# nmonette/TO-UED

Measured on NVIDIA B200. Metric: gridworld agent env-steps/sec incl. LPG update, higher is better.
Workload: dtype f16/bf16 operands, f32 accumulate (GRU); f32 elsewhere

## Files before the change

__graft_entry__.py:

```python
import os
import sys

ROOT = os.path.dirname(os.path.abspath(__file__))
if ROOT not in sys.path:
    sys.path.insert(0, ROOT)


def build() -> None:
    from to_ued_b200.csrc.build import build as _build
    path = _build(verbose=False)
    _build(verbose=False, variant="fuzz")
    import to_ued_b200
    from to_ued_b200 import _lib
    assert os.path.exists(path) and _lib.lib().toued_version() >= 1


def smoke() -> None:
    import numpy as np
    import torch
    sys.path.insert(0, os.path.join(ROOT, "tests"))
    from helpers import Case, to_oracle_traj, rel_err
    from oracle import prng
    from oracle.agents import AgentTables
    from oracle.meta import lpg_meta_grad_train_step as o_step
    from to_ued_b200.meta.train import lpg_meta_grad_train_step, LPGTrainState, _WS_CACHE
    from to_ued_b200.models.lpg import LPG
    from to_ued_b200.models.optim import Adam
    from to_ued_b200.util.data import LpgHyperparams, TrainState

    assert torch.cuda.is_available(), "smoke() needs cuda:0"
    torch.cuda.set_device(0)
    K, n = 2, 2
    c = Case("all_shortlife", n=n, seed=1, table_scale=0.3)
    ag, ro = c.agent_state()
    ts = LPGTrainState(LPG(), torch.from_numpy(c.lpg).cuda(), Adam(1e-4))
    vc = TrainState(Case.pad8(c.value), torch.zeros(n, dtype=torch.int32, device="cuda"), 1, 4e0, 0.5)
    hy = LpgHyperparams(K, 0.5, 5e-2, 1e-3, 5e-3, 1e-3)
    new_ts, ag2, vc2, met = lpg_meta_grad_train_step(prng.PRNGKey(3), ts, ag, vc, ro, 1, 0.99, 0.95, hy, return_grad=True)
    torch.cuda.synchronize()
    tape = list(_WS_CACHE.values())[0].tape
    trajs = [to_oracle_traj(tape.transition(k)) for k in range(K)]
    ev = to_oracle_traj(tape.transition(K))
    s0 = c.oro.batch_reset(None, c.p, c.w)
    rngs = prng.split(prng.PRNGKey(3), n)
    r_train = prng.split(rngs, 2)[:, 1, :]
    r0 = prng.split(r_train, 2)[:, 1, :]
    otraj, _, _ = c.oro.batch_rollout(r0, c.actor, c.p, s0)
    assert (otraj.action == trajs[0].action).all() and (otraj.obs_idx == trajs[0].obs_idx).all(), "rollout parity"
    dt = torch.float64
    oag = AgentTables(torch.tensor(c.actor).to(dt), torch.tensor(c.critic).to(dt), torch.zeros(n, dtype=torch.long))
    o = o_step(prng.PRNGKey(3), c.layout, torch.tensor(c.lpg).to(dt), oag, torch.tensor(c.value).to(dt), c.oro, c.p,
               s0, c.life, num_agent_updates=K, trajectories=trajs, eval_trajectory=ev, do_eval=False)
    err = rel_err(met["_grad"].cpu().numpy(), o["grad"].numpy())
    import to_ued_b200
    tol = 2e-2 if to_ued_b200.GRU_PRECISION == "tc" else 2e-4
    assert err < tol, f"meta-gradient mismatch vs oracle: {err}"
    print(f"smoke ok: rollout bit-exact, meta-gradient rel err {err:.2e}, lpg_loss {float(met['lpg_loss']):.5f}")


if __name__ == "__main__":
    build()
    if "--smoke" in sys.argv:
        smoke()
```

include/toued.h:

```cpp
#ifndef TOUED_H
#define TOUED_H
#include <stdint.h>
#ifdef __cplusplus
extern "C" {
#endif

#define TOUED_LEVEL_BYTES 192

const char* toued_last_error(void);
int toued_version(void);

int toued_rollout(const void* levels, const uint32_t* keys, const float* actor,
                  const uint8_t* forced_actions, int32_t* state, int32_t* obs, uint8_t* action,
                  float* reward, uint8_t* done, float* ep_return, int n_agents, int n_workers,
                  int rollout_len, int obs_dim, int max_grid_size, int max_n_objs, int reset_first,
                  void* stream);

int toued_env_step(const void* levels, const uint32_t* keys, const int32_t* actions, int32_t* state,
                   int32_t* obs, float* reward, uint8_t* done, int n_agents, int n_workers,
                   int max_grid_size, int max_n_objs, void* stream);
int toued_env_reset(const void* levels, int32_t* state, int32_t* obs, int n_agents, int n_workers,
                    int max_grid_size, void* stream);


int toued_sort_tokens(const int32_t* obs, uint16_t* sorted_tok, int n_agents, int n_workers,
                      int rollout_len, void* stream);

int toued_lpg_prepare(const int32_t* obs, const uint8_t* action, const float* reward,
                      const uint8_t* done, const float* actor, const float* critic,
                      const float* lpg_params, const int32_t* step, const void* levels, float* x,
                      void* ximg, int n_agents, int n_workers, int rollout_len, int obs_dim,
                      int lifetime_conditioning, int lpg_stride, void* stream);

int toued_gru_forward(const float* x, const uint8_t* done, const float* lpg_params, float* h_out,
                      float* gates, float* pi_hat, float* y_hat, int n_agents, int n_workers,
                      int rollout_len, int lifetime_conditioning, int lpg_stride, void* stream);

int toued_agent_scratch_floats(int n_agents, int n_workers, int rollout_len, int obs_dim);
int toued_agent_update(const int32_t* obs, const uint8_t* action, const uint16_t* sorted_tok,
                       const float* pi_hat, const float* y_hat, const float* actor_in,
                       const float* critic_in, float* actor_out, float* critic_out,
                       const void* levels, int32_t* step, float* scalars, int n_agents,
                       int n_workers, int rollout_len, int obs_dim, float lr_actor, float lr_critic,
                       float max_grad_norm, float agent_target_coeff, int tables_precopied, float* run_scratch,
                       void* stream);


int toued_meta_loss(const int32_t* obs, const uint8_t* action, const float* reward,
                    const uint8_t* done, const uint16_t* sorted_tok, const float* value_table,
                    const float* actor, float* lam, float* mu, float* scalars, int n_agents,
                    int n_workers, int rollout_len, int obs_dim, int value_stride, float gamma,
                    float gae_lambda, float grad_scale, int outer_product_quirk, void* stream);

int toued_agent_backward(const int32_t* obs, const uint8_t* action, const uint16_t* sorted_tok,
                         const float* pi_hat, const float* y_hat, const float* actor_k,
                         const float* critic_k, const float* actor_k1, const float* critic_k1,
                         const float* update_scalars, float* lam, float* mu, float* d_pi_hat,
                         float* d_y_hat, int n_agents, int n_workers, int rollout_len, int obs_dim,
                         float lr_actor, float lr_critic, float max_grad_norm,
                         float agent_target_coeff, float policy_entropy_coeff,
                         float target_entropy_coeff, float policy_l2_coeff, float target_l2_coeff,
                         float grad_scale, float* run_scratch, void* stream);

int toued_transpose_wh(const float* lpg_params, float* whT, void* stream);

int toued_gru_backward(const uint8_t* done, const float* lpg_params, const float* whT,
                       const float* h, float* gates, const float* y_hat, const float* d_pi_hat,
                       const float* d_y_hat, float* dl, float* dx, int n_agents, int n_workers,
                       int rollout_len, int lifetime_conditioning, void* stream);

int toued_lpg_wgrad_workspace_floats(void);
int toued_lpg_wgrad(const int32_t* obs, const uint8_t* done, const float* critic,
                    const float* lpg_params, const float* x, const float* h, const float* dgates,
                    const float* d_pi_hat, const float* dl, const float* dx, float* workspace,
                    int n_agents, int n_workers, int rollout_len, int obs_dim,
                    int lifetime_conditioning, int accumulate, void* stream);
int toued_lpg_wgrad_workspace_offset(int which);
int toued_lpg_wgrad_embed(const int32_t* obs, const uint8_t* done, const float* critic, const float* lpg_params,
                          const float* dx, float* workspace, const uint32_t* cotangent_max, int n_agents, int n_workers,
                          int rollout_len, int obs_dim, int lifetime_conditioning, int accumulate, void* stream);
int toued_lpg_wgrad_splits(int which);
int toued_reduce_partials(const float* workspace, float* grad, int lifetime_conditioning, int wh_splits,
                          int sm_splits, void* stream);

int toued_adam(float* params, const float* grad, float* mu, float* nu, int n, int count, float lr,
               float b1, float b2, float eps, void* stream);
int toued_adam_dev(float* params, const float* grad, float* mu, float* nu, int* count_dev, int n, float lr,
                   float b1, float b2, float eps, void* stream);
int toued_sgd_clip(float* params, const float* grad, float* sqnorm_scratch, int n, float lr, float max_norm,
                   void* stream);

int toued_a2c_update(const int32_t* obs, const uint8_t* action, const float* reward, const uint8_t* done,
                     const uint16_t* sorted_tok, const float* actor_in, const float* critic_in,
                     float* actor_out, float* critic_out, const void* levels, int32_t* step,
                     float* scalars, int n_agents, int n_workers, int rollout_len, int obs_dim,
                     float lr_actor, float lr_critic, float max_grad_norm, float gamma, float gae_lambda,
                     float entropy_coeff, int outer_product_quirk, void* stream);

int toued_a2c_train(const void* levels, const uint32_t* keys, float* actor0, float* actor1, float* critic0,
                    float* critic1, int32_t* state, int32_t* obs, uint8_t* action, float* reward, uint8_t* done,
                    uint16_t* sorted_tok, int32_t* step, float* scalars, float* loss_sums, int num_updates,
                    int n_agents, int n_workers, int rollout_len, int obs_dim, int max_grid_size, int max_n_objs,
                    float lr_actor, float lr_critic, float max_grad_norm, float gamma, float gae_lambda,
                    float entropy_coeff, int outer_product_quirk, void* stream);

int toued_es_ask(const uint32_t* key, const float* mean, float sigma, float* candidates, int popsize,
                 int n_params, int cand_stride, void* stream);
int toued_es_tell(const float* candidates, const float* fitness, float* mean, float* m, float* v,
                  int popsize, int n_params, int cand_stride, float sigma, float lrate, float beta1,
                  float beta2, float eps, int gen_counter, float mean_decay, void* stream);

int toued_es_ask_shard(const uint32_t* key, const float* mean, float sigma, float* candidates, int popsize_global,
                       int n_params, int cand_stride, int pair_offset, int n_pairs, void* stream);
int toued_es_grad_partial(const float* candidates, const float* fitness, const float* mean, float* grad_sum,
                          int n_members, int n_params, int cand_stride, float sigma, void* stream);
int toued_es_adam(const float* grad_sum, float* mean, float* m, float* v, int popsize_global, int n_params,
                  float sigma, float lrate, float beta1, float beta2, float eps, int gen_counter, float mean_decay,
                  void* stream);

int toued_plr_reset_lowest(float* score, uint8_t* active, uint8_t* is_new, int buffer_size, int minimum_new,
                           int* reset_ids, void* stream);
int toued_plr_select(uint32_t key0, uint32_t key1, float* score, uint8_t* active, uint8_t* is_new, int buffer_size,
                     const int* old_ids, const uint8_t* terminated, const float* new_scores, int n_agents,
                     float p_replay, float temperature, int shuffle_rounds, int* new_ids, void* stream);

int toued_generate_levels_desc_bytes(void);
int toued_generate_levels(const void* gen_desc, const uint32_t* keys, const int32_t* buffer_ids, void* levels_out,
                          int32_t* lifetimes_out, int n_levels, void* stream);

int toued_get_nash(const float* game, const float* x0, const float* y0, float* x_out, float* y_out,
                   int n, int x_nz, int y_nz, int num_iters, float lr, void* stream);
int toued_projection_simplex(float* v, int n, int max_nz, void* stream);


int toued_init_tables(const uint32_t* keys, const uint8_t* mask, float* tables, int n_agents,
                      int obs_dim, int n_out, void* stream);
int toued_masked_reset(const void* levels, const uint8_t* mask, int32_t* state, int32_t* obs,
                       int32_t* step, int n_agents, int n_workers, int max_grid_size, void* stream);

int toued_host_iota_bits(const uint32_t* keys, int n_keys, int n, uint32_t* out);


int toued_key_split(const uint32_t* keys_in, int n_keys, int num, int offset, int count, uint32_t* out,
                    void* stream);
int toued_key_chain(const uint32_t* keys_in, int n_keys, int chain_len, uint32_t* keys_out,
                    uint32_t* carry_out, void* stream);


int toued_tc_gemm_test(const float* A, const float* B, void* scratch_img, float* D, void* stream);
int toued_tc_gemm_mixed_test(const float* A, const float* B, void* scratch_img, float* D, void* stream);
int toued_tc_gemm_mn_test(const float* A, const float* B, void* scratch_img, float* D, int lbo, int sbo,
                          int kadv, void* stream);
int toued_tc_gemm_mn2_test(const float* A, const float* B, void* scratch_img, float* D, void* stream);

int toued_pack_wh_forward(const float* lpg_params, void* wh_img, int lifetime_conditioning, void* stream);
int toued_gru_forward_tc(const float* x, const uint8_t* done, const float* lpg_params, const void* wh_img,
                         void* h16, void* fac, void* hpimg, float* pi_hat, float* y_hat, int n_agents,
                         int n_workers, int rollout_len, int lifetime_conditioning, void* stream);
int toued_pack_wh_forward_multi(const float* lpg_params, void* wh_img, int lifetime_conditioning, int n_sets,
                                int lpg_stride, void* stream);
int toued_gru_forward_tc_multi(const float* x, const uint8_t* done, const float* lpg_params, const void* wh_img,
                               float* pi_hat, float* y_hat, int n_agents, int n_workers, int rollout_len,
                               int lifetime_conditioning, int lpg_stride, void* stream);

int toued_pack_wh_backward(const float* lpg_params, void* whb_img, void* stream);
#define TOUED_STATUS_NONFINITE_COT 1u
#define TOUED_STATUS_FP16_RANGE 2u
int toued_cotangent_max(const float* d_pi_hat, const float* d_y_hat, int n_agents, int n_workers, int rollout_len,
                        uint32_t* cotangent_max, void* stream);
int toued_gru_backward_tc(const uint8_t* done, const float* lpg_params, const void* whb_img,
                          const void* h16, const void* fac, const float* y_hat, const float* d_pi_hat,
                          const float* d_y_hat, void* dgimg, float* dl, float* dx, uint32_t* cotangent_max,
                          int n_agents, int n_workers, int rollout_len, int lifetime_conditioning, void* stream);
int toued_wgrad_tc_splits(void);
int toued_wgrad_tc_small_splits(void);
int toued_lpg_wgrad_tc(const void* hpimg, const void* dgimg, const void* ximg, const void* h16,
                       const float* d_pi_hat, const float* dl, float* wh_partials, float* small_partials,
                       uint32_t* cotangent_max, int n_agents, int n_workers, int rollout_len, int accumulate,
                       void* stream);

#ifdef __cplusplus
}
#endif
#endif
```

to_ued_b200/_lib.py:

```python
from __future__ import annotations

import ctypes as C
import os

_HERE = os.path.dirname(os.path.abspath(__file__))
_VARIANT = os.environ.get("TOUED_LIB_VARIANT", "")
LIB_PATH = os.path.join(_HERE, f"libtoued_{_VARIANT}.so" if _VARIANT else "libtoued.so")

_lib = None


class TouedError(RuntimeError):
    pass


def lib() -> C.CDLL:
    global _lib
    if _lib is None:
        if not os.path.exists(LIB_PATH):
            raise TouedError(
                f"{LIB_PATH} is missing: the CUDA extension is not built. "
                "Run `python -m to_ued_b200.csrc.build` (there is no CPU fallback).")
        _lib = C.CDLL(LIB_PATH)
        _declare(_lib)
    return _lib


_P, _I, _F = C.c_void_p, C.c_int, C.c_float

SIGNATURES = {
    "toued_rollout": [_P] * 10 + [_I] * 7 + [_P],
    "toued_env_step": [_P] * 7 + [_I] * 4 + [_P],
    "toued_env_reset": [_P] * 3 + [_I] * 3 + [_P],
    "toued_sort_tokens": [_P] * 2 + [_I] * 3 + [_P],
    "toued_lpg_prepare": [_P] * 11 + [_I] * 6 + [_P],
    "toued_gru_forward": [_P] * 7 + [_I] * 5 + [_P],
    "toued_agent_update": [_P] * 12 + [_I] * 4 + [_F] * 4 + [_I, _P, _P],
    "toued_agent_scratch_floats": [_I] * 4,
    "toued_meta_loss": [_P] * 10 + [_I] * 5 + [_F] * 3 + [_I, _P],
    "toued_agent_backward": [_P] * 14 + [_I] * 4 + [_F] * 9 + [_P, _P],
    "toued_transpose_wh": [_P] * 3,
    "toued_gru_backward": [_P] * 10 + [_I] * 4 + [_P],
    "toued_lpg_wgrad_workspace_floats": [],
    "toued_lpg_wgrad": [_P] * 11 + [_I] * 6 + [_P],
    "toued_reduce_partials": [_P, _P, _I, _I, _I, _P],
    "toued_lpg_wgrad_splits": [_I],
    "toued_lpg_wgrad_workspace_offset": [_I],
    "toued_lpg_wgrad_embed": [_P] * 7 + [_I] * 6 + [_P],
    "toued_cotangent_max": [_P, _P, _I, _I, _I, _P, _P],
    "toued_pack_wh_backward": [_P] * 3,
    "toued_gru_backward_tc": [_P] * 12 + [_I] * 4 + [_P],
    "toued_wgrad_tc_splits": [],
    "toued_wgrad_tc_small_splits": [],
    "toued_lpg_wgrad_tc": [_P] * 9 + [_I] * 4 + [_P],
    "toued_adam": [_P] * 4 + [_I, _I] + [_F] * 4 + [_P],
    "toued_adam_dev": [_P] * 5 + [_I] + [_F] * 4 + [_P],
    "toued_sgd_clip": [_P] * 3 + [_I, _F, _F, _P],
    "toued_get_nash": [_P] * 5 + [_I] * 4 + [_F, _P],
    "toued_projection_simplex": [_P, _I, _I, _P],
    "toued_es_ask": [_P, _P, _F, _P, _I, _I, _I, _P],
    "toued_es_tell": [_P] * 5 + [_I, _I, _I] + [_F] * 5 + [_I, _F, _P],
    "toued_es_ask_shard": [_P, _P, _F, _P, _I, _I, _I, _I, _I, _P],
    "toued_es_grad_partial": [_P] * 4 + [_I, _I, _I, _F, _P],
    "toued_es_adam": [_P] * 4 + [_I, _I] + [_F] * 5 + [_I, _F, _P],
    "toued_a2c_update": [_P] * 12 + [_I] * 4 + [_F] * 6 + [_I, _P],
    "toued_a2c_train": [_P] * 15 + [_I] * 7 + [_F] * 6 + [_I, _P],
    "toued_init_tables": [_P] * 3 + [_I] * 3 + [_P],
    "toued_masked_reset": [_P] * 5 + [_I] * 3 + [_P],
    "toued_generate_levels_desc_bytes": [],
    "toued_generate_levels": [_P] * 5 + [_I, _P],
    "toued_plr_reset_lowest": [_P] * 3 + [_I, _I, _P, _P],
    "toued_plr_select": [C.c_uint32, C.c_uint32] + [_P] * 3 + [_I] + [_P] * 3 + [_I, _F, _F, _I, _P, _P],
    "toued_tc_gemm_test": [_P] * 5,
    "toued_tc_gemm_mixed_test": [_P] * 5,
    "toued_tc_gemm_mn_test": [_P] * 4 + [_I] * 3 + [_P],
    "toued_tc_gemm_mn2_test": [_P] * 5,
    "toued_pack_wh_forward": [_P, _P, _I, _P],
    "toued_pack_wh_forward_multi": [_P, _P, _I, _I, _I, _P],
    "toued_gru_forward_tc_multi": [_P] * 6 + [_I] * 5 + [_P],
    "toued_host_iota_bits": [_P, _I, _I, _P],
    "toued_key_split": [_P, _I, _I, _I, _I, _P, _P],
    "toued_key_chain": [_P, _I, _I, _P, _P, _P],
    "toued_gru_forward_tc": [_P] * 9 + [_I] * 4 + [_P],
}


def _declare(l):
    l.toued_last_error.restype = C.c_char_p
    l.toued_last_error.argtypes = []
    l.toued_version.restype = _I
    l.toued_version.argtypes = []
    for name, args in SIGNATURES.items():
        fn = getattr(l, name)
        fn.restype = _I
        fn.argtypes = args


def ptr(t):
    if t is None:
        return None
    if not t.is_cuda:
        raise TouedError("to_ued_b200 ops need CUDA tensors (there is no CPU fallback)")
    if not t.is_contiguous():
        raise TouedError("to_ued_b200 ops need contiguous tensors")
    return t.data_ptr()


def stream_ptr():
    import torch
    return torch.cuda.current_stream().cuda_stream


KERNELS_PER_CALL = {"toued_adam_dev": 2, "toued_sgd_clip": 2, "toued_lpg_wgrad": 3, "toued_init_tables": 2, "toued_lpg_wgrad_tc": 2, "toued_pack_wh_forward": 2, "toued_pack_wh_forward_multi": 2}
LAUNCHES = {}
GRAPH_KERNELS = [0]
ENV_STEPS = [0]
PROFILE = None


H2D_BYTES = [0]


def h2d(t):
    H2D_BYTES[0] += int(t.numel() * t.element_size()) if hasattr(t, "element_size") else int(t.nbytes)
    return t


def reset_counters(profile=False):
    global PROFILE
    H2D_BYTES[0] = 0
    GRAPH_KERNELS[0] = 0
    ENV_STEPS[0] = 0
    LAUNCHES.clear()
    PROFILE = {} if profile else None


def kernel_launches():
    return sum(n * KERNELS_PER_CALL.get(k, 1) for k, n in LAUNCHES.items()) + GRAPH_KERNELS[0]


def profile_ms():
    return {k: (len(v), sum(a.elapsed_time(b) for a, b in v)) for k, v in (PROFILE or {}).items()}


def call(name, *args):
    LAUNCHES[name] = LAUNCHES.get(name, 0) + 1
    if name == "toued_rollout":
        ENV_STEPS[0] += args[10] * args[11] * args[12]
    elif name == "toued_a2c_train":
        ENV_STEPS[0] += args[15] * args[16] * args[17] * args[18]
    if PROFILE is not None:
        import torch
        a, b = torch.cuda.Event(enable_timing=True), torch.cuda.Event(enable_timing=True)
        a.record()
        rc = getattr(lib(), name)(*args)
        b.record()
        PROFILE.setdefault(name, []).append((a, b))
    else:
        rc = getattr(lib(), name)(*args)
    if rc != 0:
        raise TouedError(f"{name} failed ({rc}): {lib().toued_last_error().decode()}")
```

to_ued_b200/agents/lpg_agent.py:

```python
from __future__ import annotations

from dataclasses import dataclass, field
from typing import Any, List, Optional

import numpy as np
import torch

from .. import _lib
from ..util import prng
from ..util.data import AgentState, Transition


@dataclass
class LPGAgentMetrics:
    policy_l2: Any
    policy_entropy: Any
    critic_loss: Any
    critic_l2: Any
    critic_entropy: Any

    def as_dict(self):
        return {"policy_l2": self.policy_l2, "policy_entropy": self.policy_entropy,
                "critic_loss": self.critic_loss, "critic_l2": self.critic_l2,
                "critic_entropy": self.critic_entropy}


class Tape:

    def __init__(self, n_agents, n_workers, rollout_len, obs_dim, num_updates, device, keep_gates=True,
                 precision=None, per_agent_params=False):
        import to_ued_b200
        N, W, L, D, K = n_agents, n_workers, rollout_len, obs_dim, num_updates
        R, dev = N * W, device
        f32, u8, i32 = torch.float32, torch.uint8, torch.int32
        self.N, self.W, self.L, self.D, self.K, self.R = N, W, L, D, K, R
        self.record = bool(keep_gates)
        kt = K + 1 if self.record else 2
        kr = K + 1 if self.record else 1
        ka = K if self.record else 1
        self.kt, self.kr, self.ka = kt, kr, ka
        self.actor = torch.empty((kt, N, D, 8), dtype=f32, device=dev)
        self.critic = torch.empty((kt, N, D, 8), dtype=f32, device=dev)
        self.obs = torch.empty((kr, N, L + 1, W), dtype=i32, device=dev)
        self.action = torch.empty((kr, N, L, W), dtype=u8, device=dev)
        self.reward = torch.empty((kr, N, L, W), dtype=f32, device=dev)
        self.done = torch.empty((kr, N, L, W), dtype=u8, device=dev)
        self.sorted_tok = torch.empty((kr, N, L * W), dtype=torch.int16, device=dev)
        self.precision = precision or to_ued_b200.GRU_PRECISION
        self.x = torch.empty((ka, L, R, 8), dtype=f32, device=dev)
        self.ximg = None
        if self.precision == "tc":
            f16 = torch.float16
            Rp = (R + 63) // 64 * 64
            R32 = (R + 31) // 32 * 32
            self.h16 = None if per_agent_params else torch.empty((ka, L, R32, 256), dtype=f16, device=dev)
            self.fac = torch.empty((ka, 4, L, R32, 256), dtype=f16, device=dev) if self.record else None
            self.hpimg = torch.zeros((ka, L * Rp * 256 * 2), dtype=torch.uint8, device=dev) if self.record else None
            self.ximg = torch.zeros((ka, L * Rp * 128), dtype=torch.uint8, device=dev) if self.record else None
            self.wh_img = torch.zeros((N if per_agent_params else 1) * 16 * 26624 // 2, dtype=f16, device=dev)
            self.h = self.gates = None
        else:
            self.h = torch.empty((ka, L, R, 256), dtype=f32, device=dev)
            self.gates = torch.empty((ka, 4, L, R, 256), dtype=f32, device=dev) if self.record else None
        self.pi_hat = torch.empty((ka, L, R), dtype=f32, device=dev)
        self.y_hat = torch.empty((ka, L, R, 8), dtype=f32, device=dev)
        self.scalars = torch.empty((ka, N, 8), dtype=f32, device=dev)
        self.scal_sum = torch.zeros((N, 8), dtype=f32, device=dev)
        self.step_in = torch.empty((ka, N), dtype=i32, device=dev)
        self.ep_return = torch.empty((N, W), dtype=f32, device=dev)
        self.agent_scratch = torch.empty(_lib.lib().toued_agent_scratch_floats(N, W, L, D), dtype=f32, device=dev)

    def ti(self, k):
        return k if self.record else (k & 1)

    def ri(self, k):
        return k if self.record else 0

    def ai(self, k):
        return k if self.record else 0

    def transition(self, k) -> Transition:
        r = self.ri(k)
        return Transition(self.obs[r], self.action[r], self.reward[r], self.done[r])


_SORT_STREAMS = {}


def _sort_stream(cur):
    key = (cur.device.index, cur.cuda_stream)
    st = _SORT_STREAMS.get(key)
    if st is None:
        st = _SORT_STREAMS[key] = torch.cuda.Stream(device=cur.device)
    return st


def _mark(label):
    import to_ued_b200
    if to_ued_b200.PHASE_EVENTS is not None and getattr(to_ued_b200, "PHASE_FINE", False):
        e = torch.cuda.Event(enable_timing=True)
        e.record(torch.cuda.current_stream())
        to_ued_b200.PHASE_EVENTS.append((label, -2, e))


def lpg_agent_train_step(k, tape: Tape, levels, step, lpg_params, lifetime_conditioning, agent_target_coeff,
                         lr_actor, lr_critic, max_grad_norm, lpg_stride=0):
    N, W, L, D = tape.N, tape.W, tape.L, tape.D
    s = _lib.stream_ptr()
    p = _lib.ptr
    r, a, t0, t1 = tape.ri(k), tape.ai(k), tape.ti(k), tape.ti(k + 1)
    import to_ued_b200
    cur = torch.cuda.current_stream()
    side = _sort_stream(cur) if to_ued_b200.SIDE_STREAMS else cur
    ev_roll, ev_sort = torch.cuda.Event(), torch.cuda.Event()
    ev_roll.record(cur)
    with torch.cuda.stream(side):
        side.wait_event(ev_roll)
        _lib.call("toued_sort_tokens", p(tape.obs[r]), p(tape.sorted_tok[r]), N, W, L, _lib.stream_ptr())
        precopied = bool(to_ued_b200.SIDE_STREAMS)
        if precopied:
            tape.actor[t1].copy_(tape.actor[t0])
            tape.critic[t1].copy_(tape.critic[t0])
        ev_sort.record(side)
    _mark("rollout")
    tape.step_in[a].copy_(step)
    _lib.call("toued_lpg_prepare", p(tape.obs[r]), p(tape.action[r]), p(tape.reward[r]), p(tape.done[r]),
              p(tape.actor[t0]), p(tape.critic[t0]), p(lpg_params), p(step), p(levels), p(tape.x[a]),
              p(tape.ximg[a]) if tape.ximg is not None else None,
              N, W, L, D, int(lifetime_conditioning), int(lpg_stride), s)
    if lpg_stride and tape.precision == "tc":
        _lib.call("toued_gru_forward_tc_multi", p(tape.x[a]), p(tape.done[r]), p(lpg_params), p(tape.wh_img),
                  p(tape.pi_hat[a]), p(tape.y_hat[a]), N, W, L, int(lifetime_conditioning), int(lpg_stride), s)
    elif lpg_stride or tape.precision != "tc":
        _lib.call("toued_gru_forward", p(tape.x[a]), p(tape.done[r]), p(lpg_params), p(tape.h[a]),
                  p(tape.gates[a]) if tape.gates is not None else None, p(tape.pi_hat[a]), p(tape.y_hat[a]),
                  N, W, L, int(lifetime_conditioning), int(lpg_stride), s)
    else:
        _lib.call("toued_gru_forward_tc", p(tape.x[a]), p(tape.done[r]), p(lpg_params), p(tape.wh_img),
                  p(tape.h16[a]), p(tape.fac[a]) if tape.fac is not None else None,
                  p(tape.hpimg[a]) if tape.hpimg is not None else None, p(tape.pi_hat[a]), p(tape.y_hat[a]),
                  N, W, L, int(lifetime_conditioning), s)
    _mark("gru_fwd")
    cur.wait_event(ev_sort)
    _mark("sort_wait")
    _lib.call("toued_agent_update", p(tape.obs[r]), p(tape.action[r]), p(tape.sorted_tok[r]), p(tape.pi_hat[a]),
              p(tape.y_hat[a]), p(tape.actor[t0]), p(tape.critic[t0]), p(tape.actor[t1]), p(tape.critic[t1]),
              p(levels), p(step), p(tape.scalars[a]), N, W, L, D, float(lr_actor), float(lr_critic),
              float(max_grad_norm), float(agent_target_coeff), int(precopied), p(tape.agent_scratch), s)
    tape.scal_sum += tape.scalars[a]
    _mark("update")


def train_lpg_agent_steps(rng, lpg_train_state, agent_state: AgentState, rollout_manager, num_train_steps: int,
                          agent_target_coeff: float, tape: Optional[Tape] = None, lpg_stride: int = 0):
    env = rollout_manager.env
    actor, critic = agent_state.actor_state, agent_state.critic_state
    N, W = agent_state.env_state.packed.shape
    L, K = rollout_manager.train_rollout_len, num_train_steps
    dev = actor.params.device
    if tape is None:
        import to_ued_b200
        tape = Tape(N, W, L, env.obs_dim, K, dev, keep_gates=False,
                    precision=to_ued_b200.ES_PRECISION if lpg_stride else None, per_agent_params=bool(lpg_stride))
    levels = agent_state.level.packed
    step = actor.step.clone()
    state = agent_state.env_state.packed.clone()
    tape.actor[0].copy_(actor.params)
    tape.critic[0].copy_(critic.params)
    tape.scal_sum.zero_()
    keys_d = prng.chain_device(prng.to_device(rng, dev), K)
    p = _lib.ptr
    lpg = lpg_train_state.params if hasattr(lpg_train_state, "params") else lpg_train_state
    cond = lpg_train_state.model.lifetime_conditioning if hasattr(lpg_train_state, "model") else False
    if tape.precision == "tc" and not lpg_stride:
        _lib.call("toued_pack_wh_forward", p(lpg), p(tape.wh_img), int(cond), _lib.stream_ptr())
    elif tape.precision == "tc":
        _lib.call("toued_pack_wh_forward_multi", p(lpg), p(tape.wh_img), int(cond), N, int(lpg_stride), _lib.stream_ptr())
    yield
    for k in range(K):
        r = tape.ri(k)
        _lib.call("toued_rollout", p(levels), p(keys_d[k]), p(tape.actor[tape.ti(k)]), None, p(state), p(tape.obs[r]),
                  p(tape.action[r]), p(tape.reward[r]), p(tape.done[r]), None, N, W, L, env.obs_dim,
                  env.max_grid_size, env.max_n_objs, 0, _lib.stream_ptr())
        lpg_agent_train_step(k, tape, levels, step, lpg, cond, agent_target_coeff, actor.learning_rate,
                             critic.learning_rate, actor.max_grad_norm, lpg_stride=lpg_stride)
        yield
    sc = tape.scal_sum / K
    metrics = LPGAgentMetrics(policy_l2=sc[:, 4], policy_entropy=sc[:, 6], critic_loss=sc[:, 3],
                              critic_l2=sc[:, 5], critic_entropy=sc[:, 7])
    from ..environments.gridworld.gridworld import EnvState
    new_agent = agent_state.replace(
        actor_state=actor.replace(params=tape.actor[tape.ti(K)].clone(), step=step),
        critic_state=critic.replace(params=tape.critic[tape.ti(K)].clone(), step=step.clone()),
        env_obs=tape.obs[tape.ri(K - 1)][:, -1].clone(), env_state=EnvState(state, env.max_n_objs))
    rollouts = [tape.transition(k) for k in range(K)] if tape.record else [tape.transition(K - 1)]
    return new_agent, rollouts, metrics


def train_lpg_agent(rng, lpg_train_state, agent_state: AgentState, rollout_manager, num_train_steps: int,
                    agent_target_coeff: float, tape: Optional[Tape] = None, lpg_stride: int = 0):
    gen = train_lpg_agent_steps(rng, lpg_train_state, agent_state, rollout_manager, num_train_steps,
                                agent_target_coeff, tape=tape, lpg_stride=lpg_stride)
    while True:
        try:
            next(gen)
        except StopIteration as done:
            return done.value
```

to_ued_b200/csrc/agent_backward.cu:

```cuda
#include "lpg_common.cuh"
#include "segreduce.cuh"
#include "../../include/toued.h"

__global__ void __launch_bounds__(256)
meta_loss_kernel(const int32_t* __restrict__ obs, const uint8_t* __restrict__ action,
                 const float* __restrict__ reward, const uint8_t* __restrict__ done,
                 const uint16_t* __restrict__ sorted_tok, const float* __restrict__ value,
                 const float* __restrict__ actor, float* __restrict__ lam, float* __restrict__ mu,
                 float* __restrict__ scal, int W, int L, int D, int vstride, float gamma, float lmbda,
                 float gscale, int quirk) {
    extern __shared__ __align__(16) float sm[];
    float* adv = sm;
    float* rec = adv + L * W;
    float* abar = rec + L * W * 6;
    float* lbar = abar + W;
    float* runv = lbar + W;
    float* scan = runv + L * W * 5;
    void* idxmem = scan + 2 * 256 * 5;
    __shared__ float red[32];
    __shared__ int iscan[512];
    __shared__ unsigned char sflags[512];
    const int n = blockIdx.x, tid = threadIdx.x, T = W * L;
    const int32_t* ob = obs + (size_t)n * (L + 1) * W;
    const uint8_t* act = action + (size_t)n * T;
    const float* rw = reward + (size_t)n * T;
    const uint8_t* dn = done + (size_t)n * T;
    const uint16_t* st = sorted_tok + (size_t)n * T;
    const float* vt = value + (size_t)n * D * vstride;
    const float* at = actor + (size_t)n * D * 8;
    float* lm = lam + (size_t)n * D * 8;
    float* mm = mu + (size_t)n * D * 8;
    const float invT = 1.0f / (float)T;
    const SegIndex si = seg_index_build(idxmem, iscan, st, ob, T);

    for (int i = tid; i < D * 2; i += 256) {
        reinterpret_cast<float4*>(lm)[i] = make_float4(0.f, 0.f, 0.f, 0.f);
        reinterpret_cast<float4*>(mm)[i] = make_float4(0.f, 0.f, 0.f, 0.f);
    }
    float s1 = 0.f, s2 = 0.f;
    const float vlast = vt[(size_t)(D - 1) * vstride];
    for (int w = tid; w < W; w += 256) {
        float g = 0.f;
        int32_t o1 = ob[L * W + w];
        float v1 = vt[(size_t)ob_idx(o1) * vstride] + 0.001f * (float)ob_time(o1) * vlast;
        for (int t = L - 1; t >= 0; --t) {
            const int32_t o0 = ob[t * W + w];
            const float v0 = vt[(size_t)ob_idx(o0) * vstride] + 0.001f * (float)ob_time(o0) * vlast;
            const float nd = dn[t * W + w] ? 0.0f : 1.0f;
            const float delta = rw[t * W + w] + gamma * v1 * nd - v0;
            g = delta + gamma * lmbda * nd * g;
            adv[t * W + w] = g;
            s1 += g; s2 = fmaf(g, g, s2);
            v1 = v0;
        }
    }
    s1 = block_sum(s1, red); s2 = block_sum(s2, red);
    const float mean = s1 * invT;
    float var = 0.f;
    for (int i = tid; i < T; i += 256) { const float d = adv[i] - mean; var = fmaf(d, d, var); }
    var = block_sum(var, red) * invT;
    const float inv_std = 1.0f / (sqrtf(var) + 1e-8f);
    __syncthreads();
    for (int i = tid; i < T; i += 256) adv[i] = (adv[i] - mean) * inv_std;
    __syncthreads();
    for (int tok = tid; tok < T; tok += 256) {
        const int32_t o = ob[tok];
        float z[5], p[5];
        tab_logits8<5>(at, D, o, z);
        softmax_c<5>(z, p);
        const int a = act[tok];
        float pa = p[0];
#pragma unroll
        for (int j = 1; j < 5; ++j) pa = (a == j) ? p[j] : pa;
        float* r = rec + tok * 6;
        r[5] = logf(pa + 1e-8f);
        const float q = pa / (pa + 1e-8f);
#pragma unroll
        for (int j = 0; j < 5; ++j) r[j] = q * ((a == j ? 1.0f : 0.0f) - p[j]);
    }
    __syncthreads();
    float loss = 0.f;
    for (int w = tid; w < W; w += 256) {
        float sa = 0.f, sl = 0.f, se = 0.f;
        for (int t = 0; t < L; ++t) { sa += adv[t * W + w]; sl += rec[(t * W + w) * 6 + 5]; se = fmaf(adv[t * W + w], rec[(t * W + w) * 6 + 5], se); }
        abar[w] = sa / (float)L; lbar[w] = sl / (float)L;
        loss -= quirk ? abar[w] * lbar[w] : se / (float)L;
    }
    loss = block_sum(loss, red) / (float)W;
    __syncthreads();
    float last[5] = {0.f, 0.f, 0.f, 0.f, 0.f};
    for (int tok = tid; tok < T; tok += 256) {
        const int w = tok % W;
        const float coef = -gscale * invT * (quirk ? abar[w] : adv[tok]);
        float* r = rec + tok * 6;
        const float tf = 0.001f * (float)ob_time(ob[tok]);
#pragma unroll
        for (int j = 0; j < 5; ++j) { r[j] *= coef; last[j] = fmaf(tf, r[j], last[j]); }
        r[5] = tf;
    }
#pragma unroll
    for (int j = 0; j < 5; ++j) last[j] = block_sum(last[j], red);
    __syncthreads();
    seg_reduce<5, 6>(rec, si, T, runv, scan, sflags);
    for (int r = tid; r < si.nruns; r += 256) {
        const int row = si.run_row[r];
#pragma unroll
        for (int j = 0; j < 5; ++j) lm[(size_t)row * 8 + j] = runv[r * 5 + j];
    }
    if (tid == 0) {
#pragma unroll
        for (int j = 0; j < 5; ++j) lm[(size_t)(D - 1) * 8 + j] = last[j];
        scal[n * 2 + 0] = loss;
        scal[n * 2 + 1] = s2 * invT;
    }
}

extern "C" int toued_meta_loss(const int32_t* obs, const uint8_t* action, const float* reward,
                               const uint8_t* done, const uint16_t* sorted_tok, const float* value_table,
                               const float* actor, float* lam, float* mu, float* scalars, int n_agents,
                               int n_workers, int rollout_len, int obs_dim, int value_stride, float gamma,
                               float gae_lambda, float grad_scale, int outer_product_quirk, void* stream) {
    const int T = n_workers * rollout_len;
    TOUED_CHECK(n_agents > 0 && T > 0, "toued_meta_loss: empty problem");
    const size_t smem = sizeof(float) * ((size_t)T * 7 + 2 * n_workers + (size_t)T * 5 + 2 * 256 * 5) + seg_index_bytes(T);
    TOUED_CHECK(smem <= 200 * 1024, "toued_meta_loss: W*L=%d too large for shared memory", T);
    TOUED_CUDA(cudaFuncSetAttribute(meta_loss_kernel, cudaFuncAttributeMaxDynamicSharedMemorySize, (int)smem));
    meta_loss_kernel<<<n_agents, 256, smem, (cudaStream_t)stream>>>(
        obs, action, reward, done, sorted_tok, value_table, actor, lam, mu, scalars, n_workers, rollout_len,
        obs_dim, value_stride, gamma, gae_lambda, grad_scale, outer_product_quirk);
    TOUED_LAUNCH_CHECK();
    return 0;
}

struct TokFwd { float p[5], y[8], pa, q, tf; int a; };

__device__ __forceinline__ TokFwd tok_forward(const float* at, const float* ct, int D, int32_t o, int a) {
    TokFwd f;
    float z[5], zy[8];
    tab_logits8<5>(at, D, o, z);
    softmax_c<5>(z, f.p);
    tab_logits8<8>(ct, D, o, zy);
    softmax_c<8>(zy, f.y);
    f.a = a;
    f.pa = f.p[0];
#pragma unroll
    for (int j = 1; j < 5; ++j) f.pa = (a == j) ? f.p[j] : f.pa;
    f.q = f.pa / (f.pa + 1e-8f);
    f.tf = 0.001f * (float)ob_time(o);
    return f;
}

__device__ __forceinline__ void tok_grad(const TokFwd& f, float ph, const float* yh, float invT, float alpha, float* c) {
    const float ca = invT * ph * f.q;
#pragma unroll
    for (int j = 0; j < 5; ++j) c[j] = ca * ((f.a == j ? 1.0f : 0.0f) - f.p[j]);
    float mm[8], b = 0.f;
#pragma unroll
    for (int i = 0; i < 8; ++i) {
        mm[i] = logf(f.y[i] + 1e-8f) - logf(yh[i] + 1e-8f) + f.y[i] / (f.y[i] + 1e-8f);
        b = fmaf(f.y[i], mm[i], b);
    }
    const float cc = alpha * invT;
#pragma unroll
    for (int i = 0; i < 8; ++i) c[5 + i] = cc * f.y[i] * (mm[i] - b);
}

__device__ __forceinline__ void load8(const float* p, float* v) {
    const float4 a = reinterpret_cast<const float4*>(p)[0], b = reinterpret_cast<const float4*>(p)[1];
    v[0] = a.x; v[1] = a.y; v[2] = a.z; v[3] = a.w; v[4] = b.x; v[5] = b.y; v[6] = b.z; v[7] = b.w;
}

__global__ void __launch_bounds__(256, 2)
agent_backward_kernel(const int32_t* __restrict__ obs, const uint8_t* __restrict__ action,
                      const uint16_t* __restrict__ sorted_tok, const float* __restrict__ pi_hat,
                      const float* __restrict__ y_hat, const float* __restrict__ actor_k,
                      const float* __restrict__ critic_k, const float* __restrict__ actor_k1,
                      const float* __restrict__ critic_k1, const float* __restrict__ upd_scal,
                      float* lam, float* mu, float* __restrict__ d_pi_hat, float* __restrict__ d_y_hat,
                      float* run_scratch, int n_agents, int W, int L, int D, float lr_a, float lr_c, float max_norm,
                      float alpha, float b_pent, float b_yent, float b_pl2, float b_yl2, float gscale) {
    extern __shared__ __align__(16) float rec[];
    __shared__ float red[32];
    __shared__ float s_wlast[13];
    __shared__ int iscan[512];
    __shared__ unsigned char sflags[512];
    const int n = blockIdx.x, tid = threadIdx.x, T = W * L, R = n_agents * W;
    const int32_t* ob = obs + (size_t)n * (L + 1) * W;
    const uint8_t* act = action + (size_t)n * T;
    const uint16_t* st = sorted_tok + (size_t)n * T;
    const float* a0 = actor_k + (size_t)n * D * 8;
    const float* c0 = critic_k + (size_t)n * D * 8;
    const float* a1 = actor_k1 + (size_t)n * D * 8;
    const float* c1 = critic_k1 + (size_t)n * D * 8;
    float* lm = lam + (size_t)n * D * 8;
    float* mm = mu + (size_t)n * D * 8;
    const float invT = 1.0f / (float)T;
    const float gna = upd_scal[n * 8 + 0], gnc = upd_scal[n * 8 + 1];
    const bool keep = upd_scal[n * 8 + 2] != 0.0f;
    float* runv = run_scratch + (size_t)n * min(T, D) * 13;
    float* scan = rec + (size_t)T * 13;
    const SegIndex si = seg_index_build(scan + 2 * 256 * 13, iscan, st, ob, T);

    float last[13];
#pragma unroll
    for (int j = 0; j < 13; ++j) last[j] = 0.f;
    for (int tok = tid; tok < T; tok += 256) {
        const TokFwd f = tok_forward(a1, c1, D, ob[tok], act[tok]);
        float* r = rec + tok * 13;
        {
            float dh[5], s = 0.f;
#pragma unroll
            for (int j = 0; j < 5; ++j) { dh[j] = -(logf(f.p[j] + 1e-8f) + 1.0f); s = fmaf(f.p[j], dh[j], s); }
            const float k = -b_pent * gscale * invT;
#pragma unroll
            for (int j = 0; j < 5; ++j) r[j] = k * f.p[j] * (dh[j] - s);
        }
        {
            float dh[8], s = 0.f;
#pragma unroll
            for (int j = 0; j < 8; ++j) { dh[j] = -(logf(f.y[j] + 1e-8f) + 1.0f); s = fmaf(f.y[j], dh[j], s); }
            const float k = -b_yent * gscale * invT;
#pragma unroll
            for (int j = 0; j < 8; ++j) r[5 + j] = k * f.y[j] * (dh[j] - s);
        }
#pragma unroll
        for (int j = 0; j < 13; ++j) last[j] = fmaf(f.tf, r[j], last[j]);
    }
#pragma unroll
    for (int j = 0; j < 13; ++j) last[j] = block_sum(last[j], red);
    __syncthreads();
    seg_reduce<13, 13>(rec, si, T, runv, scan, sflags);
    for (int r = tid; r < si.nruns; r += 256) {
        const int row = si.run_row[r];
        const float* g = runv + r * 13;
#pragma unroll
        for (int j = 0; j < 5; ++j) lm[(size_t)row * 8 + j] += g[j];
#pragma unroll
        for (int j = 0; j < 8; ++j) mm[(size_t)row * 8 + j] += g[5 + j];
    }
    if (tid == 0) {
#pragma unroll
        for (int j = 0; j < 5; ++j) lm[(size_t)(D - 1) * 8 + j] += last[j];
#pragma unroll
        for (int j = 0; j < 8; ++j) mm[(size_t)(D - 1) * 8 + j] += last[5 + j];
    }
    __syncthreads();

    const float dir_pi = gscale * b_pl2 * 2.0f * invT;
    const float dir_y = gscale * b_yl2 * 2.0f * invT;
    if (!keep) {
        for (int tok = tid; tok < T; tok += 256) {
            const int t = tok / W, w = tok - t * W;
            const size_t li = (size_t)t * R + (size_t)n * W + w;
            d_pi_hat[li] = dir_pi * pi_hat[li];
            float yh[8]; load8(y_hat + li * 8, yh);
            float4* o = reinterpret_cast<float4*>(d_y_hat + li * 8);
            o[0] = make_float4(dir_y * yh[0], dir_y * yh[1], dir_y * yh[2], dir_y * yh[3]);
            o[1] = make_float4(dir_y * yh[4], dir_y * yh[5], dir_y * yh[6], dir_y * yh[7]);
        }
        return;
    }

#pragma unroll
    for (int j = 0; j < 13; ++j) last[j] = 0.f;
    for (int tok = tid; tok < T; tok += 256) {
        const int t = tok / W, w = tok - t * W;
        const size_t li = (size_t)t * R + (size_t)n * W + w;
        const TokFwd f = tok_forward(a0, c0, D, ob[tok], act[tok]);
        float yh[8]; load8(y_hat + li * 8, yh);
        float* r = rec + tok * 13;
        tok_grad(f, pi_hat[li], yh, invT, alpha, r);
#pragma unroll
        for (int j = 0; j < 13; ++j) last[j] = fmaf(f.tf, r[j], last[j]);
    }
#pragma unroll
    for (int j = 0; j < 13; ++j) last[j] = block_sum(last[j], red);
    __syncthreads();
    seg_reduce<13, 13>(rec, si, T, runv, scan, sflags);
    float dot_a = 0.f, dot_c = 0.f;
    for (int r = tid; r < si.nruns; r += 256) {
        const int row = si.run_row[r];
        const float* g = runv + r * 13;
        float l8[8], m8[8];
        load8(lm + (size_t)row * 8, l8); load8(mm + (size_t)row * 8, m8);
#pragma unroll
        for (int j = 0; j < 5; ++j) dot_a = fmaf(g[j], l8[j], dot_a);
#pragma unroll
        for (int j = 0; j < 8; ++j) dot_c = fmaf(g[5 + j], m8[j], dot_c);
    }
    dot_a = block_sum(dot_a, red); dot_c = block_sum(dot_c, red);
    float ll[8], ml[8];
    load8(lm + (size_t)(D - 1) * 8, ll); load8(mm + (size_t)(D - 1) * 8, ml);
#pragma unroll
    for (int j = 0; j < 5; ++j) dot_a = fmaf(last[j], ll[j], dot_a);
#pragma unroll
    for (int j = 0; j < 8; ++j) dot_c = fmaf(last[5 + j], ml[j], dot_c);
    const bool clip_a = !(gna < max_norm), clip_c = !(gnc < max_norm);
    const float ka = -lr_a * (clip_a ? max_norm / gna : 1.0f), pa_ = clip_a ? dot_a / (gna * gna) : 0.0f;
    const float kc = -lr_c * (clip_c ? max_norm / gnc : 1.0f), pc_ = clip_c ? dot_c / (gnc * gnc) : 0.0f;
    if (tid == 0) {
#pragma unroll
        for (int j = 0; j < 5; ++j) s_wlast[j] = ka * (ll[j] - pa_ * last[j]);
#pragma unroll
        for (int j = 0; j < 8; ++j) s_wlast[5 + j] = kc * (ml[j] - pc_ * last[5 + j]);
    }
    __syncthreads();
    float wl[13];
#pragma unroll
    for (int j = 0; j < 13; ++j) wl[j] = s_wlast[j];

    for (int r = tid; r < si.nruns; r += 256) {
        const int row = si.run_row[r];
        float* g = runv + r * 13;
        float l8[8], m8[8];
        load8(lm + (size_t)row * 8, l8); load8(mm + (size_t)row * 8, m8);
#pragma unroll
        for (int j = 0; j < 5; ++j) g[j] = ka * (l8[j] - pa_ * g[j]);
#pragma unroll
        for (int j = 0; j < 8; ++j) g[5 + j] = kc * (m8[j] - pc_ * g[5 + j]);
    }
    __syncthreads();
    float hl[13];
#pragma unroll
    for (int j = 0; j < 13; ++j) hl[j] = 0.f;
    for (int pos = tid; pos < T; pos += 256) {
        const int tok = si.tok[pos];
        const int t = tok / W, w = tok - t * W;
        const size_t li = (size_t)t * R + (size_t)n * W + w;
        const TokFwd f = tok_forward(a0, c0, D, ob[tok], act[tok]);
        const float ph = pi_hat[li];
        float yh[8]; load8(y_hat + li * 8, yh);
        float* r = rec + tok * 13;
        const float* wr = runv + (size_t)si.run[pos] * 13;
        float v[13];
#pragma unroll
        for (int j = 0; j < 13; ++j) v[j] = fmaf(f.tf, wl[j], wr[j]);
        float va = v[0], pv = 0.f;
#pragma unroll
        for (int j = 1; j < 5; ++j) va = (f.a == j) ? v[j] : va;
#pragma unroll
        for (int j = 0; j < 5; ++j) pv = fmaf(f.p[j], v[j], pv);
        const float s = va - pv;
        d_pi_hat[li] = invT * f.q * s + dir_pi * ph;
        const float pe = f.pa + 1e-8f;
        const float c1_ = ph * invT * s * 1e-8f * f.pa / (pe * pe), c2_ = ph * invT * f.q;
        float h[13];
#pragma unroll
        for (int j = 0; j < 5; ++j)
            h[j] = c1_ * ((f.a == j ? 1.0f : 0.0f) - f.p[j]) - c2_ * f.p[j] * (v[j] - pv);
        float m[8], mp[8], av = 0.f, b = 0.f;
#pragma unroll
        for (int j = 0; j < 8; ++j) {
            const float ye = f.y[j] + 1e-8f;
            m[j] = logf(ye) - logf(yh[j] + 1e-8f) + f.y[j] / ye;
            mp[j] = (f.y[j] + 2e-8f) / (ye * ye);
            av = fmaf(v[5 + j], f.y[j], av);
            b = fmaf(f.y[j], m[j], b);
        }
        const float ca = alpha * invT;
        float dS[8], sy = 0.f, dyo[8];
#pragma unroll
        for (int j = 0; j < 8; ++j) {
            const float vc = v[5 + j];
            dyo[j] = ca * f.y[j] * (av - vc) / (yh[j] + 1e-8f) + dir_y * yh[j];
            dS[j] = vc * m[j] + vc * f.y[j] * mp[j] - vc * b - av * (m[j] + f.y[j] * mp[j]);
            sy = fmaf(f.y[j], dS[j], sy);
        }
#pragma unroll
        for (int j = 0; j < 8; ++j) h[5 + j] = ca * f.y[j] * (dS[j] - sy);
        float4* o = reinterpret_cast<float4*>(d_y_hat + li * 8);
        o[0] = make_float4(dyo[0], dyo[1], dyo[2], dyo[3]);
        o[1] = make_float4(dyo[4], dyo[5], dyo[6], dyo[7]);
#pragma unroll
        for (int j = 0; j < 13; ++j) { r[j] = h[j]; hl[j] = fmaf(f.tf, h[j], hl[j]); }
    }
#pragma unroll
    for (int j = 0; j < 13; ++j) hl[j] = block_sum(hl[j], red);
    __syncthreads();
    seg_reduce<13, 13>(rec, si, T, runv, scan, sflags);
    for (int r = tid; r < si.nruns; r += 256) {
        const int row = si.run_row[r];
        const float* g = runv + r * 13;
#pragma unroll
        for (int j = 0; j < 5; ++j) lm[(size_t)row * 8 + j] += g[j];
#pragma unroll
        for (int j = 0; j < 8; ++j) mm[(size_t)row * 8 + j] += g[5 + j];
    }
    if (tid == 0) {
#pragma unroll
        for (int j = 0; j < 5; ++j) lm[(size_t)(D - 1) * 8 + j] = ll[j] + hl[j];
#pragma unroll
        for (int j = 0; j < 8; ++j) mm[(size_t)(D - 1) * 8 + j] = ml[j] + hl[5 + j];
    }
}

extern "C" int toued_agent_backward(const int32_t* obs, const uint8_t* action, const uint16_t* sorted_tok,
                                    const float* pi_hat, const float* y_hat, const float* actor_k,
                                    const float* critic_k, const float* actor_k1, const float* critic_k1,
                                    const float* update_scalars, float* lam, float* mu, float* d_pi_hat,
                                    float* d_y_hat, int n_agents, int n_workers, int rollout_len, int obs_dim,
                                    float lr_actor, float lr_critic, float max_grad_norm,
                                    float agent_target_coeff, float policy_entropy_coeff,
                                    float target_entropy_coeff, float policy_l2_coeff, float target_l2_coeff,
                                    float grad_scale, float* run_scratch, void* stream) {
    const int T = n_workers * rollout_len;
    TOUED_CHECK(n_agents > 0 && T > 0, "toued_agent_backward: empty problem");
    TOUED_CHECK(run_scratch != nullptr, "toued_agent_backward: run_scratch (toued_agent_scratch_floats) is required");
    const size_t smem = sizeof(float) * ((size_t)T * 13 + 2 * 256 * 13) + seg_index_bytes(T);
    TOUED_CHECK(smem <= 200 * 1024, "toued_agent_backward: W*L=%d too large for shared memory", T);
    TOUED_CUDA(cudaFuncSetAttribute(agent_backward_kernel, cudaFuncAttributeMaxDynamicSharedMemorySize, (int)smem));
    TOUED_CUDA(cudaFuncSetAttribute(agent_backward_kernel, cudaFuncAttributePreferredSharedMemoryCarveout, 100));
    cudaStream_t st = (cudaStream_t)stream;
    agent_backward_kernel<<<n_agents, 256, smem, st>>>(
        obs, action, sorted_tok, pi_hat, y_hat, actor_k, critic_k, actor_k1, critic_k1, update_scalars, lam, mu,
        d_pi_hat, d_y_hat, run_scratch, n_agents, n_workers, rollout_len, obs_dim, lr_actor, lr_critic, max_grad_norm,
        agent_target_coeff, policy_entropy_coeff, target_entropy_coeff, policy_l2_coeff, target_l2_coeff, grad_scale);
    TOUED_LAUNCH_CHECK();
    return 0;
}
```

to_ued_b200/csrc/agent_update.cu:

```cuda
#include "lpg_common.cuh"
#include "segreduce.cuh"
#include "../../include/toued.h"

constexpr int AU_C = 13;

__global__ void __launch_bounds__(256, 2)
agent_update_kernel(const int32_t* __restrict__ obs, const uint8_t* __restrict__ action,
                    const uint16_t* __restrict__ sorted_tok, const float* __restrict__ pi_hat,
                    const float* __restrict__ y_hat, const float* __restrict__ actor_in,
                    const float* __restrict__ critic_in, float* actor_out, float* critic_out,
                    const LevelRec* __restrict__ levels, int32_t* __restrict__ step,
                    float* __restrict__ scal, float* run_scratch, int n_agents, int W, int L, int D,
                    float lr_a, float lr_c, float max_norm, float alpha, int tables_precopied) {
    extern __shared__ __align__(16) float smc[];
    __shared__ float red[32];
    __shared__ int iscan[512];
    __shared__ unsigned char sflags[512];
    const int n = blockIdx.x, tid = threadIdx.x, T = W * L, R = n_agents * W;
    float* runv = run_scratch + (size_t)n * min(T, D) * 13;
    float* scan = smc + (size_t)T * AU_C;
    void* idxmem = scan + 2 * 256 * 13;
    const int32_t* ob = obs + (size_t)n * (L + 1) * W;
    const uint8_t* act = action + (size_t)n * T;
    const float* a_in = actor_in + (size_t)n * D * 8;
    const float* c_in = critic_in + (size_t)n * D * 8;
    float* a_out = actor_out + (size_t)n * D * 8;
    float* c_out = critic_out + (size_t)n * D * 8;
    const float invT = 1.0f / (float)T;
    const SegIndex si = seg_index_build(idxmem, iscan, sorted_tok + (size_t)n * T, ob, T);

    if (!tables_precopied)
        for (int i = tid; i < D * 2; i += 256) {
            reinterpret_cast<float4*>(a_out)[i] = reinterpret_cast<const float4*>(a_in)[i];
            reinterpret_cast<float4*>(c_out)[i] = reinterpret_cast<const float4*>(c_in)[i];
        }

    float m_kl = 0.f, m_pi2 = 0.f, m_y2 = 0.f;
    float last[13];
#pragma unroll
    for (int j = 0; j < 13; ++j) last[j] = 0.f;
    for (int tok = tid; tok < T; tok += 256) {
        const int t = tok / W, w = tok - t * W;
        const size_t li = (size_t)t * R + (size_t)n * W + w;
        const int32_t o = ob[tok];
        float z[5], p[5], zy[8], y[8];
        tab_logits8<5>(a_in, D, o, z);
        softmax_c<5>(z, p);
        tab_logits8<8>(c_in, D, o, zy);
        softmax_c<8>(zy, y);
        const int a = act[tok];
        float pa = p[0];
#pragma unroll
        for (int j = 1; j < 5; ++j) pa = (a == j) ? p[j] : pa;
        const float ph = pi_hat[li];
        const float ca = invT * ph * (pa / (pa + 1e-8f));
        float* rec = smc + tok * AU_C;
#pragma unroll
        for (int j = 0; j < 5; ++j) rec[j] = ca * ((a == j ? 1.0f : 0.0f) - p[j]);
        float yh[8];
        { const float4* q = reinterpret_cast<const float4*>(y_hat + li * 8); const float4 q0 = q[0], q1 = q[1];
          yh[0] = q0.x; yh[1] = q0.y; yh[2] = q0.z; yh[3] = q0.w; yh[4] = q1.x; yh[5] = q1.y; yh[6] = q1.z; yh[7] = q1.w; }
        float mm[8], b = 0.f, kl = 0.f, y2 = 0.f;
#pragma unroll
        for (int i = 0; i < 8; ++i) {
            const float ly = logf(y[i] + 1e-8f), lh = logf(yh[i] + 1e-8f);
            mm[i] = ly - lh + y[i] / (y[i] + 1e-8f);
            b = fmaf(y[i], mm[i], b);
            kl = fmaf(y[i], ly - lh, kl);
            y2 = fmaf(yh[i], yh[i], y2);
        }
        const float cc = alpha * invT;
#pragma unroll
        for (int i = 0; i < 8; ++i) rec[5 + i] = cc * y[i] * (mm[i] - b);
        const float tf = 0.001f * (float)ob_time(o);
#pragma unroll
        for (int j = 0; j < 13; ++j) last[j] = fmaf(tf, rec[j], last[j]);
        m_kl += kl; m_pi2 = fmaf(ph, ph, m_pi2); m_y2 += y2;
    }
#pragma unroll
    for (int j = 0; j < 13; ++j) last[j] = block_sum(last[j], red);
    m_kl = block_sum(m_kl, red); m_pi2 = block_sum(m_pi2, red); m_y2 = block_sum(m_y2, red);
    __syncthreads();

    seg_reduce<13, AU_C>(smc, si, T, runv, scan, sflags);
    float na = 0.f, nc = 0.f;
    for (int r = tid; r < si.nruns; r += 256) {
        const float* g = runv + r * 13;
#pragma unroll
        for (int j = 0; j < 5; ++j) na = fmaf(g[j], g[j], na);
#pragma unroll
        for (int j = 5; j < 13; ++j) nc = fmaf(g[j], g[j], nc);
    }
    na = block_sum(na, red); nc = block_sum(nc, red);
#pragma unroll
    for (int j = 0; j < 5; ++j) na = fmaf(last[j], last[j], na);
#pragma unroll
    for (int j = 5; j < 13; ++j) nc = fmaf(last[j], last[j], nc);
    const float gna = sqrtf(na), gnc = sqrtf(nc);
    const float sa = gna < max_norm ? 1.0f : max_norm / gna;
    const float sc = gnc < max_norm ? 1.0f : max_norm / gnc;
    const int old_step = step[n];
    const bool keep = (old_step + 1) <= levels[n].lifetime;
    const float ua = keep ? lr_a * sa : 0.0f, uc = keep ? lr_c * sc : 0.0f;

    for (int r = tid; r < si.nruns; r += 256) {
        const int row = si.run_row[r];
        const float* g = runv + r * 13;
#pragma unroll
        for (int j = 0; j < 5; ++j) a_out[(size_t)row * 8 + j] = a_in[(size_t)row * 8 + j] - ua * g[j];
#pragma unroll
        for (int j = 0; j < 8; ++j) c_out[(size_t)row * 8 + j] = c_in[(size_t)row * 8 + j] - uc * g[5 + j];
    }
    if (tid == 0) {
#pragma unroll
        for (int j = 0; j < 5; ++j) a_out[(size_t)(D - 1) * 8 + j] = a_in[(size_t)(D - 1) * 8 + j] - ua * last[j];
#pragma unroll
        for (int j = 0; j < 8; ++j) c_out[(size_t)(D - 1) * 8 + j] = c_in[(size_t)(D - 1) * 8 + j] - uc * last[5 + j];
        step[n] = keep ? old_step + 1 : old_step;
    }
    __syncthreads();

    float ea = 0.f, ec = 0.f;
    for (int tok = tid; tok < T; tok += 256) {
        const int32_t o = ob[tok];
        float z[5], p[5], zy[8], y[8];
        tab_logits8<5>(a_out, D, o, z);
        softmax_c<5>(z, p);
        tab_logits8<8>(c_out, D, o, zy);
        softmax_c<8>(zy, y);
#pragma unroll
        for (int j = 0; j < 5; ++j) { const float q = p[j] + 1e-8f; ea -= q * logf(q); }
#pragma unroll
        for (int j = 0; j < 8; ++j) { const float q = y[j] + 1e-8f; ec -= q * logf(q); }
    }
    ea = block_sum(ea, red); ec = block_sum(ec, red);
    if (tid == 0) {
        float* s = scal + (size_t)n * 8;
        s[0] = gna; s[1] = gnc; s[2] = keep ? 1.0f : 0.0f;
        s[3] = m_kl * invT;
        s[4] = m_pi2 * invT;
        s[5] = m_y2 * invT;
        s[6] = ea * invT;
        s[7] = ec * invT;
    }
}

static size_t agent_smem_bytes(int T, int D) {
    return sizeof(float) * ((size_t)T * AU_C + 2 * 256 * 13) + seg_index_bytes(T);
}

extern "C" int toued_agent_update(const int32_t* obs, const uint8_t* action, const uint16_t* sorted_tok,
                                  const float* pi_hat, const float* y_hat, const float* actor_in,
                                  const float* critic_in, float* actor_out, float* critic_out,
                                  const void* levels, int32_t* step, float* scalars, int n_agents,
                                  int n_workers, int rollout_len, int obs_dim, float lr_actor,
                                  float lr_critic, float max_grad_norm, float agent_target_coeff, int tables_precopied,
                                  float* run_scratch, void* stream) {
    const int T = n_workers * rollout_len;
    const size_t smem = agent_smem_bytes(T, obs_dim);
    TOUED_CHECK(n_agents > 0 && T > 0, "toued_agent_update: empty problem");
    TOUED_CHECK(smem <= 200 * 1024, "toued_agent_update: W*L=%d too large for shared memory", T);
    TOUED_CHECK(actor_in != actor_out && critic_in != critic_out, "toued_agent_update: in-place update not supported");
    TOUED_CUDA(cudaFuncSetAttribute(agent_update_kernel, cudaFuncAttributeMaxDynamicSharedMemorySize, (int)smem));
    TOUED_CUDA(cudaFuncSetAttribute(agent_update_kernel, cudaFuncAttributePreferredSharedMemoryCarveout, 100));
    TOUED_CHECK(run_scratch != nullptr, "toued_agent_update: run_scratch (toued_agent_scratch_floats) is required");
    cudaStream_t st = (cudaStream_t)stream;
    agent_update_kernel<<<n_agents, 256, smem, st>>>(
        obs, action, sorted_tok, pi_hat, y_hat, actor_in, critic_in, actor_out, critic_out,
        (const LevelRec*)levels, step, scalars, run_scratch, n_agents, n_workers, rollout_len, obs_dim,
        lr_actor, lr_critic, max_grad_norm, agent_target_coeff, tables_precopied);
    TOUED_LAUNCH_CHECK();
    return 0;
}

extern "C" int toued_agent_scratch_floats(int n_agents, int n_workers, int rollout_len, int obs_dim) {
    const long long T = (long long)n_workers * rollout_len;
    const long long n = 13ll * (T < obs_dim ? T : obs_dim) * n_agents;
    return n < (1ll << 31) ? (int)n : -1;
}
```

to_ued_b200/csrc/build.py:

```python
import os, subprocess, sys, hashlib, shutil

HERE = os.path.dirname(os.path.abspath(__file__))
OUT = os.path.join(HERE, "..", "libtoued.so")
ARCH = ["-gencode", "arch=compute_100a,code=sm_100a"]
COMMON = ["-O3", "-lineinfo", "-std=c++17", "-Xcompiler", "-fPIC"]
FLAGS = {
    "rollout.cu": ["-O3", "-lineinfo", "-std=c++17", "-Xcompiler", "-fPIC", "-fmad=false"],
    "levelgen.cu": ["-O3", "-lineinfo", "-std=c++17", "-Xcompiler", "-fPIC", "-fmad=false"],
}


def _nvcc():
    return shutil.which("nvcc") or "/usr/local/cuda/bin/nvcc"


VARIANTS = {
    "probe": ["-DTOUED_RACE_PROBE=1"],
    "fuzz": ["-DTOUED_FUZZ=1"],
    "fuzz_old": ["-DTOUED_FUZZ=1", "-DTOUED_XTILE_OLD=1"],
    "bwd16": ["-DBT_EW=16"],
    "wgpair": ["-DTOUED_WGRAD_PAIR=1"],
    "wpprobe": ["-DTOUED_WGRAD_PAIR=1", "-DTOUED_WP_PROBE=1"],
    "wgk": ["-DTOUED_WGRAD_KMAJOR=1"],
    "fwdns7": ["-DFT_NS_OVERRIDE=7"],
    "fwd1": ["-DFT_HEADS_WARP=0"],
    "pf2": ["-DBT_PF_DEPTH=2"],
    "pf": ["-DBT_L2_PREFETCH=1"],
    "old": ["-DTOUED_XTILE_OLD=1"],
    "probe_old": ["-DTOUED_RACE_PROBE=1", "-DTOUED_XTILE_OLD=1"],
}


def build(verbose=False, force=False, variant=""):
    global OUT
    if variant:
        return _build(verbose, force, os.path.join(HERE, "..", f"libtoued_{variant}.so"),
                      os.path.join(HERE, f"build_{variant}"), VARIANTS[variant])
    return _build(verbose, force, OUT, os.path.join(HERE, "build"), [])


def _build(verbose, force, OUT, objdir, extra):
    srcs = sorted(f for f in os.listdir(HERE) if f.endswith(".cu"))
    hdrs = sorted(f for f in os.listdir(HERE) if f.endswith(".cuh")) + ["../../include/toued.h"]
    hsig = hashlib.sha1(b"".join(open(os.path.join(HERE, h), "rb").read() for h in hdrs)).hexdigest()
    os.makedirs(objdir, exist_ok=True)
    objs, rebuilt = [], False
    for s in srcs:
        src = os.path.join(HERE, s)
        obj = os.path.join(objdir, s[:-3] + ".o")
        flags = list(FLAGS.get(s, COMMON)) + list(extra)
        sig = hashlib.sha1(open(src, "rb").read() + hsig.encode() + " ".join(flags).encode()).hexdigest()
        sigf = obj + ".sig"
        if force or not os.path.exists(obj) or not os.path.exists(sigf) or open(sigf).read() != sig:
            cmd = [_nvcc(), *ARCH, *flags, "-c", src, "-o", obj]
            if verbose:
                cmd.insert(1, "-Xptxas"); cmd.insert(2, "-v")
                print(" ".join(cmd), flush=True)
            subprocess.check_call(cmd)
            open(sigf, "w").write(sig)
            rebuilt = True
        objs.append(obj)
    if rebuilt or not os.path.exists(OUT):
        cmd = [_nvcc(), *ARCH, "-shared", "-o", OUT, *objs, "-lcudart"]
        if verbose:
            print(" ".join(cmd), flush=True)
        subprocess.check_call(cmd)
    return os.path.abspath(OUT)


if __name__ == "__main__":
    var = [a.split("=", 1)[1] for a in sys.argv if a.startswith("--variant=")]
    print(build(verbose="-v" in sys.argv, force="-f" in sys.argv, variant=var[0] if var else ""))
```

to_ued_b200/csrc/lpg_common.cuh:

```cuda
#pragma once
#include "common.cuh"

constexpr int LPG_H = 256;
constexpr int LPG_Y = 8;
constexpr int LPG_E = 16;
constexpr int LPG_G = 3 * LPG_H;
constexpr int LPG_XP = 8;

struct LpgOffsets {
    int e_w0, e_b0, e_w1, e_b1, Wi, bi, Wh, bhn, w_pi, b_pi, W_y, b_y, total;
};
__host__ __device__ inline LpgOffsets lpg_offsets(int X) {
    LpgOffsets o; int p = 0;
    o.Wh = p; p += LPG_H * LPG_G;
    o.Wi = p; p += X * LPG_G;
    o.bi = p; p += LPG_G;
    o.bhn = p; p += LPG_H;
    o.w_pi = p; p += LPG_H;
    o.W_y = p; p += LPG_H * LPG_Y;
    o.b_y = p; p += LPG_Y;
    o.e_w0 = p; p += LPG_Y * LPG_E;
    o.e_b0 = p; p += LPG_E;
    o.e_w1 = p; p += LPG_E;
    o.e_b1 = p; p += 1;
    o.b_pi = p; p += 1;
    o.total = p;
    return o;
}

__device__ __forceinline__ float sigmoidf_(float x) { return 1.0f / (1.0f + __expf(-x)); }
__device__ __forceinline__ float tanhf_(float x) {
    const float e = __expf(2.0f * x);
    return 1.0f - 2.0f / (e + 1.0f);
}

__device__ __forceinline__ float ex2_approx(float x) { float y; asm("ex2.approx.ftz.f32 %0, %1;" : "=f"(y) : "f"(x)); return y; }
__device__ __forceinline__ float rcp_approx(float x) { float y; asm("rcp.approx.ftz.f32 %0, %1;" : "=f"(y) : "f"(x)); return y; }
__device__ __forceinline__ float tanh_mufu(float x) { float y; asm("tanh.approx.f32 %0, %1;" : "=f"(y) : "f"(x)); return y; }
__device__ __forceinline__ float sigmoid_mufu(float x) { return fmaf(0.5f, tanh_mufu(0.5f * x), 0.5f); }
__device__ __forceinline__ float sigmoid_fast(float x) { return rcp_approx(1.0f + ex2_approx(-1.4426950408889634f * x)); }
__device__ __forceinline__ float tanh_fast(float x) { return fmaf(2.0f, rcp_approx(1.0f + ex2_approx(-2.8853900817779268f * x)), -1.0f); }

__device__ __forceinline__ float fmin_nan(float a, float b) { float r; asm("min.NaN.f32 %0, %1, %2;" : "=f"(r) : "f"(a), "f"(b)); return r; }
__device__ __forceinline__ float fmax_nan(float a, float b) { float r; asm("max.NaN.f32 %0, %1, %2;" : "=f"(r) : "f"(a), "f"(b)); return r; }
__device__ __forceinline__ float fmax3_nan(float a, float b, float c) {
    float r; asm("max.NaN.f32 %0, %1, %2, %3;" : "=f"(r) : "f"(a), "f"(b), "f"(c)); return r;
}

template <int C>
__device__ __forceinline__ void softmax_c(const float (&z)[C], float (&p)[C]) {
    float m = z[0];
#pragma unroll
    for (int j = 1; j < C; ++j) m = fmaxf(m, z[j]);
    float s = 0.0f;
#pragma unroll
    for (int j = 0; j < C; ++j) { p[j] = __expf(z[j] - m); s += p[j]; }
    const float inv = 1.0f / s;
#pragma unroll
    for (int j = 0; j < C; ++j) p[j] *= inv;
}

template <int C>
__device__ __forceinline__ void tab_logits8(const float* table, int D, int32_t ob, float (&z)[C]) {
    const float tf = 0.001f * (float)ob_time(ob);
    const float4* row = reinterpret_cast<const float4*>(table + (size_t)ob_idx(ob) * 8);
    const float4* last = reinterpret_cast<const float4*>(table + (size_t)(D - 1) * 8);
    float r[8], l[8];
    const float4 a0 = row[0], a1 = row[1], b0 = last[0], b1 = last[1];
    r[0] = a0.x; r[1] = a0.y; r[2] = a0.z; r[3] = a0.w; r[4] = a1.x; r[5] = a1.y; r[6] = a1.z; r[7] = a1.w;
    l[0] = b0.x; l[1] = b0.y; l[2] = b0.z; l[3] = b0.w; l[4] = b1.x; l[5] = b1.y; l[6] = b1.z; l[7] = b1.w;
#pragma unroll
    for (int j = 0; j < C; ++j) z[j] = r[j] + tf * l[j];
}

__device__ __forceinline__ float block_sum(float v, float* red) {
#pragma unroll
    for (int o = 16; o > 0; o >>= 1) v += __shfl_xor_sync(0xffffffffu, v, o);
    const int lane = threadIdx.x & 31, warp = threadIdx.x >> 5, nw = (blockDim.x + 31) >> 5;
    __syncthreads();
    if (lane == 0) red[warp] = v;
    __syncthreads();
    float t = (lane < nw) ? red[lane] : 0.0f;
#pragma unroll
    for (int o = 16; o > 0; o >>= 1) t += __shfl_xor_sync(0xffffffffu, t, o);
    return t;
}
```

to_ued_b200/csrc/lpg_forward.cu:

```cuda
#include "lpg_common.cuh"
#include "tc.cuh"
#include "../../include/toued.h"

template <int E>
__device__ __forceinline__ void sort_cmpx(uint32_t& mine, uint32_t other, bool keep_min) {
    const uint32_t lo = min(mine, other), hi = max(mine, other);
    mine = keep_min ? lo : hi;
}

template <int E>
__global__ void __launch_bounds__(256)
sort_tokens_reg_kernel(const int32_t* __restrict__ obs, uint16_t* __restrict__ sorted_tok, int W, int L, int T) {
    constexpr int P2 = 256 * E;
    __shared__ uint32_t xch[P2];
    const int n = blockIdx.x, tid = threadIdx.x, base = tid * E;
    const int32_t* ob = obs + (size_t)n * (L + 1) * W;
    uint32_t v[E];
#pragma unroll
    for (int e = 0; e < E; ++e) {
        const int i = base + e;
        v[e] = i < T ? ((uint32_t)ob_idx(ob[i]) << 12) | (uint32_t)i : 0xFFFFFFFFu;
    }
    for (int k = 2; k <= P2; k <<= 1) {
        for (int j = k >> 1; j >= 32 * E; j >>= 1) {
#pragma unroll
            for (int e = 0; e < E; ++e) xch[base + e] = v[e];
            __syncthreads();
#pragma unroll
            for (int e = 0; e < E; ++e) {
                const int i = base + e;
                sort_cmpx<E>(v[e], xch[i ^ j], ((i & j) == 0) == ((i & k) == 0));
            }
            __syncthreads();
        }
        for (int j = min(k >> 1, 16 * E); j >= E; j >>= 1) {
            const int lane_mask = j / E;
#pragma unroll
            for (int e = 0; e < E; ++e) {
                const int i = base + e;
                const uint32_t other = __shfl_xor_sync(0xffffffffu, v[e], lane_mask);
                sort_cmpx<E>(v[e], other, ((i & j) == 0) == ((i & k) == 0));
            }
        }
#pragma unroll
        for (int j = E / 2; j > 0; j >>= 1) {
            if (j < k) {
#pragma unroll
                for (int e = 0; e < E; ++e) {
                    if ((e & j) == 0) {
                        const bool up = ((base + e) & k) == 0;
                        const uint32_t a = v[e], b = v[e | j];
                        const uint32_t lo = min(a, b), hi = max(a, b);
                        v[e] = up ? lo : hi;
                        v[e | j] = up ? hi : lo;
                    }
                }
            }
        }
    }
#pragma unroll
    for (int e = 0; e < E; ++e)
        if (base + e < T) sorted_tok[(size_t)n * T + base + e] = (uint16_t)(v[e] & 0xFFFu);
}

__global__ void __launch_bounds__(256)
sort_tokens_kernel(const int32_t* __restrict__ obs, uint16_t* __restrict__ sorted_tok,
                   int W, int L, int T, int P2) {
    extern __shared__ uint32_t keys[];
    const int n = blockIdx.x;
    const int32_t* ob = obs + (size_t)n * (L + 1) * W;
    for (int i = threadIdx.x; i < P2; i += blockDim.x)
        keys[i] = i < T ? ((uint32_t)ob_idx(ob[i]) << 12) | (uint32_t)i : 0xFFFFFFFFu;
    __syncthreads();
    for (int k = 2; k <= P2; k <<= 1) {
        for (int j = k >> 1; j > 0; j >>= 1) {
            for (int i = threadIdx.x; i < P2; i += blockDim.x) {
                const int ixj = i ^ j;
                if (ixj > i) {
                    const uint32_t a = keys[i], b = keys[ixj];
                    const bool up = (i & k) == 0;
                    if ((a > b) == up) { keys[i] = b; keys[ixj] = a; }
                }
            }
            __syncthreads();
        }
    }
    for (int i = threadIdx.x; i < T; i += blockDim.x)
        sorted_tok[(size_t)n * T + i] = (uint16_t)(keys[i] & 0xFFFu);
}

extern "C" int toued_sort_tokens(const int32_t* obs, uint16_t* sorted_tok, int n_agents, int n_workers,
                                 int rollout_len, void* stream) {
    const int T = n_workers * rollout_len;
    TOUED_CHECK(T > 0 && T <= 4096, "toued_sort_tokens: W*L=%d must be in 1..4096", T);
    int P2 = 1; while (P2 < T) P2 <<= 1;
    cudaStream_t st = (cudaStream_t)stream;
    switch (P2) {
        case 512:  sort_tokens_reg_kernel<2><<<n_agents, 256, 0, st>>>(obs, sorted_tok, n_workers, rollout_len, T); break;
        case 1024: sort_tokens_reg_kernel<4><<<n_agents, 256, 0, st>>>(obs, sorted_tok, n_workers, rollout_len, T); break;
        case 2048: sort_tokens_reg_kernel<8><<<n_agents, 256, 0, st>>>(obs, sorted_tok, n_workers, rollout_len, T); break;
        case 4096: sort_tokens_reg_kernel<16><<<n_agents, 256, 0, st>>>(obs, sorted_tok, n_workers, rollout_len, T); break;
        default:   sort_tokens_kernel<<<n_agents, 256, P2 * sizeof(uint32_t), st>>>(obs, sorted_tok, n_workers, rollout_len, T, P2);
    }
    TOUED_LAUNCH_CHECK();
    return 0;
}

__device__ __forceinline__ void embed_mlp2(const float (&y0)[LPG_Y], const float (&y1)[LPG_Y],
                                           const float* __restrict__ sp, float& out0, float& out1) {
    out0 = out1 = sp[LPG_Y * LPG_E + LPG_E + LPG_E];
#pragma unroll 4
    for (int e = 0; e < LPG_E; ++e) {
        float a0 = sp[LPG_Y * LPG_E + e], a1 = a0;
#pragma unroll
        for (int i = 0; i < LPG_Y; ++i) {
            const float wgt = sp[i * LPG_E + e];
            a0 = fmaf(y0[i], wgt, a0);
            a1 = fmaf(y1[i], wgt, a1);
        }
        const float w1 = sp[LPG_Y * LPG_E + LPG_E + e];
        out0 = fmaf(fmax_nan(a0, 0.0f), w1, out0);
        out1 = fmaf(fmax_nan(a1, 0.0f), w1, out1);
    }
}

__global__ void __launch_bounds__(256, 4)
lpg_prepare_kernel(const int32_t* __restrict__ obs, const uint8_t* __restrict__ action,
                   const float* __restrict__ reward, const uint8_t* __restrict__ done,
                   const float* __restrict__ actor, const float* __restrict__ critic,
                   const float* __restrict__ lpg, const int32_t* __restrict__ step,
                   const LevelRec* __restrict__ levels, float* __restrict__ x, unsigned char* __restrict__ ximg,
                   int n_agents, int W, int L, int D, int cond, int emb_off, int lpg_stride) {
    __shared__ float sp_s[LPG_Y * LPG_E + LPG_E + LPG_E + 1];
    if (lpg_stride == 0) {
        for (int i = threadIdx.x; i < LPG_Y * LPG_E + 2 * LPG_E + 1; i += blockDim.x) sp_s[i] = lpg[emb_off + i];
        __syncthreads();
    }
    const size_t g = (size_t)blockIdx.x * blockDim.x + threadIdx.x;
    const size_t total = (size_t)n_agents * L * W;
    if (g >= total) return;
    const int w = (int)(g % W);
    const int t = (int)((g / W) % L);
    const int n = (int)(g / ((size_t)W * L));
    const float* sp = lpg_stride ? lpg + (size_t)n * lpg_stride + emb_off : sp_s;
    const int32_t ob = obs[((size_t)n * (L + 1) + t) * W + w];
    const int32_t ob1 = obs[((size_t)n * (L + 1) + t + 1) * W + w];
    const float* at = actor + (size_t)n * D * 8;
    const float* ct = critic + (size_t)n * D * 8;
    float z[TOUED_NUM_ACTIONS], p[TOUED_NUM_ACTIONS];
    tab_logits8<TOUED_NUM_ACTIONS>(at, D, ob, z);
    softmax_c<TOUED_NUM_ACTIONS>(z, p);
    const int a = action[g];
    float pa = p[0];
#pragma unroll
    for (int j = 1; j < TOUED_NUM_ACTIONS; ++j) pa = (a == j) ? p[j] : pa;
    float zy[LPG_Y], y0[LPG_Y], y1[LPG_Y];
    tab_logits8<LPG_Y>(ct, D, ob, zy);
    softmax_c<LPG_Y>(zy, y0);
    tab_logits8<LPG_Y>(ct, D, ob1, zy);
    softmax_c<LPG_Y>(zy, y1);
    const float d = done[g] ? 1.0f : 0.0f;
    float pyt, pyt1;
    embed_mlp2(y0, y1, sp, pyt, pyt1);
    pyt1 *= (1.0f - d);
    const size_t row = (size_t)n * W + w;
    float4* xo = reinterpret_cast<float4*>(x + ((size_t)t * n_agents * W + row) * LPG_XP);
    xo[0] = make_float4(reward[g], d, pa + 1e-8f, pyt);
    const float4 v1 = make_float4(pyt1, cond ? (float)step[n] : 0.0f, cond ? (float)levels[n].lifetime : 0.0f, 1.0f);
    xo[1] = v1;
    if (ximg) {
        const size_t Rp = ((size_t)n_agents * W + 63) & ~(size_t)63;
        __half2 b0 = __floats2half2_rn(reward[g], d), b1 = __floats2half2_rn(pa + 1e-8f, pyt);
        __half2 b2 = __floats2half2_rn(v1.x, v1.y), b3 = __floats2half2_rn(v1.z, v1.w);
        uint4 pk;
        pk.x = *reinterpret_cast<uint32_t*>(&b0); pk.y = *reinterpret_cast<uint32_t*>(&b1);
        pk.z = *reinterpret_cast<uint32_t*>(&b2); pk.w = *reinterpret_cast<uint32_t*>(&b3);
        *reinterpret_cast<uint4*>(ximg + tile_img_offset((size_t)t * Rp + row, 1, 0)) = pk;
    }
}

extern "C" int toued_lpg_prepare(const int32_t* obs, const uint8_t* action, const float* reward,
                                 const uint8_t* done, const float* actor, const float* critic,
                                 const float* lpg_params, const int32_t* step, const void* levels,
                                 float* x, void* ximg, int n_agents, int n_workers, int rollout_len, int obs_dim,
                                 int lifetime_conditioning, int lpg_stride, void* stream) {
    const size_t total = (size_t)n_agents * rollout_len * n_workers;
    TOUED_CHECK(total > 0, "toued_lpg_prepare: empty problem");
    lpg_prepare_kernel<<<(unsigned)((total + 255) / 256), 256, 0, (cudaStream_t)stream>>>(
        obs, action, reward, done, actor, critic, lpg_params, step, (const LevelRec*)levels, x, (unsigned char*)ximg,
        n_agents, n_workers, rollout_len, obs_dim, lifetime_conditioning,
        lpg_offsets(lifetime_conditioning ? 7 : 5).e_w0, lpg_stride);
    TOUED_LAUNCH_CHECK();
    return 0;
}

constexpr int GF_TM = 64;
constexpr int GF_KC = 16;
constexpr int GF_HS = LPG_H + 4;

__device__ __forceinline__ void cp_async16(void* smem, const void* gmem) {
    asm volatile("cp.async.cg.shared.global [%0], [%1], 16;" ::"r"(smem_u32(smem)), "l"(gmem));
}
__device__ __forceinline__ void cp_async_commit() { asm volatile("cp.async.commit_group;"); }
template <int N> __device__ __forceinline__ void cp_async_wait() { asm volatile("cp.async.wait_group %0;" ::"n"(N)); }

template <int X>
__global__ void __launch_bounds__(256, 1)
gru_forward_kernel(const float* __restrict__ x, const uint8_t* __restrict__ done,
                   const float* __restrict__ lpg_base, float* __restrict__ h_out, float* __restrict__ gates,
                   float* __restrict__ pi_hat, float* __restrict__ y_hat, int R, int L, int W, int lpg_stride) {
    const float* lpg = lpg_base + (size_t)((blockIdx.x * 64) / W) * lpg_stride;
    extern __shared__ __align__(16) float sm[];
    float* hA = sm;
    float* hB = hA + GF_TM * GF_HS;
    float* Bs = hB + GF_TM * GF_HS;
    float* sWi = Bs + 2 * GF_KC * 192;
    float* sbi = sWi + X * LPG_G;
    float* sbhn = sbi + LPG_G;
    float* swp = sbhn + LPG_H;
    float* sWy = swp + LPG_H;
    float* sx = sWy + LPG_H * LPG_Y;
    __shared__ float sdone[GF_TM];
    const LpgOffsets o = lpg_offsets(X);
    const float* Wh = lpg + o.Wh;
    const int tid = threadIdx.x;
    const int row0 = blockIdx.x * GF_TM;
    const int nrows = min(GF_TM, R - row0);

    for (int i = tid; i < X * LPG_G; i += 256) sWi[i] = lpg[o.Wi + i];
    for (int i = tid; i < LPG_G; i += 256) sbi[i] = lpg[o.bi + i];
    for (int i = tid; i < LPG_H; i += 256) { sbhn[i] = lpg[o.bhn + i]; swp[i] = lpg[o.w_pi + i]; }
    for (int i = tid; i < LPG_H * LPG_Y; i += 256) sWy[i] = lpg[o.W_y + i];
    for (int i = tid; i < GF_TM * GF_HS; i += 256) hB[i] = 0.0f;
    const float b_pi = lpg[o.b_pi];
    float b_y[LPG_Y];
#pragma unroll
    for (int i = 0; i < LPG_Y; ++i) b_y[i] = lpg[o.b_y + i];
    __syncthreads();

    const int rg = tid >> 4;
    const int jg = tid & 15;

    for (int t = L - 1; t >= 0; --t) {
        { float* tmp = hA; hA = hB; hB = tmp; }
        if (tid < GF_TM) {
            const int r = row0 + tid;
            sdone[tid] = (tid < nrows && done[((size_t)(r / W) * L + t) * W + (r % W)]) ? 1.0f : 0.0f;
        }
        for (int i = tid; i < GF_TM * 2; i += 256) {
            const int r = i >> 1;
            float4 v = make_float4(0.f, 0.f, 0.f, 0.f);
            if (r < nrows) v = reinterpret_cast<const float4*>(x + ((size_t)t * R + row0 + r) * LPG_XP)[i & 1];
            reinterpret_cast<float4*>(sx + r * LPG_XP)[i & 1] = v;
        }
        __syncthreads();
        for (int i = tid; i < GF_TM * 64; i += 256) {
            const int r = i >> 6;
            if (sdone[r] != 0.0f) reinterpret_cast<float4*>(hA + r * GF_HS)[i & 63] = make_float4(0.f, 0.f, 0.f, 0.f);
        }
        __syncthreads();

        for (int jb = 0; jb < 4; ++jb) {
            float acc[4][4][3];
#pragma unroll
            for (int i = 0; i < 4; ++i)
#pragma unroll
                for (int j = 0; j < 4; ++j) { acc[i][j][0] = 0.f; acc[i][j][1] = 0.f; acc[i][j][2] = 0.f; }
            auto load_chunk = [&](int buf, int k0) {
#pragma unroll
                for (int q = 0; q < 3; ++q) {
                    const int f = tid + q * 256;
                    const int kk = f / 48, rem = f % 48, gte = rem >> 4, c4 = rem & 15;
                    cp_async16(Bs + (buf * GF_KC + kk) * 192 + gte * 64 + c4 * 4,
                               Wh + (size_t)(k0 + kk) * LPG_G + gte * LPG_H + jb * 64 + c4 * 4);
                }
                cp_async_commit();
            };
            load_chunk(0, 0);
            for (int kc = 0; kc < LPG_H / GF_KC; ++kc) {
                if (kc + 1 < LPG_H / GF_KC) { load_chunk((kc + 1) & 1, (kc + 1) * GF_KC); cp_async_wait<1>(); }
                else cp_async_wait<0>();
                __syncthreads();
                const float* bs = Bs + (kc & 1) * GF_KC * 192;
#pragma unroll
                for (int k4 = 0; k4 < GF_KC; k4 += 4) {
                    float4 a[4];
#pragma unroll
                    for (int i = 0; i < 4; ++i)
                        a[i] = *reinterpret_cast<const float4*>(hA + (rg * 4 + i) * GF_HS + kc * GF_KC + k4);
#pragma unroll
                    for (int kk = 0; kk < 4; ++kk) {
                        float4 b[3];
#pragma unroll
                        for (int gte = 0; gte < 3; ++gte)
                            b[gte] = *reinterpret_cast<const float4*>(bs + (k4 + kk) * 192 + gte * 64 + jg * 4);
#pragma unroll
                        for (int i = 0; i < 4; ++i) {
                            const float av = kk == 0 ? a[i].x : kk == 1 ? a[i].y : kk == 2 ? a[i].z : a[i].w;
#pragma unroll
                            for (int gte = 0; gte < 3; ++gte) {
                                acc[i][0][gte] = fmaf(av, b[gte].x, acc[i][0][gte]);
                                acc[i][1][gte] = fmaf(av, b[gte].y, acc[i][1][gte]);
                                acc[i][2][gte] = fmaf(av, b[gte].z, acc[i][2][gte]);
                                acc[i][3][gte] = fmaf(av, b[gte].w, acc[i][3][gte]);
                            }
                        }
                    }
                }
                __syncthreads();
            }
            const int j0 = jb * 64 + jg * 4;
#pragma unroll
            for (int i = 0; i < 4; ++i) {
                const int rl = rg * 4 + i;
                float xr[X];
#pragma unroll
                for (int q = 0; q < X; ++q) xr[q] = sx[rl * LPG_XP + q];
                float hn4[4], r4[4], z4[4], n4[4], hv[4];
#pragma unroll
                for (int j = 0; j < 4; ++j) {
                    const int u = j0 + j;
                    float gr = sbi[u], gz = sbi[LPG_H + u], gn = sbi[2 * LPG_H + u];
#pragma unroll
                    for (int q = 0; q < X; ++q) {
                        gr = fmaf(xr[q], sWi[q * LPG_G + u], gr);
                        gz = fmaf(xr[q], sWi[q * LPG_G + LPG_H + u], gz);
                        gn = fmaf(xr[q], sWi[q * LPG_G + 2 * LPG_H + u], gn);
                    }
                    const float rr = sigmoidf_(gr + acc[i][j][0]);
                    const float zz = sigmoidf_(gz + acc[i][j][1]);
                    const float hn = acc[i][j][2] + sbhn[u];
                    const float nn = tanhf_(gn + rr * hn);
                    const float hp = hA[rl * GF_HS + u];
                    r4[j] = rr; z4[j] = zz; n4[j] = nn; hn4[j] = hn;
                    hv[j] = (1.0f - zz) * nn + zz * hp;
                }
                *reinterpret_cast<float4*>(hB + rl * GF_HS + j0) = make_float4(hv[0], hv[1], hv[2], hv[3]);
                if (rl < nrows) {
                    const size_t base = ((size_t)t * R + row0 + rl) * LPG_H + j0;
                    *reinterpret_cast<float4*>(h_out + base) = make_float4(hv[0], hv[1], hv[2], hv[3]);
                    if (gates) {
                        const size_t gs = (size_t)L * R * LPG_H;
                        *reinterpret_cast<float4*>(gates + base) = make_float4(r4[0], r4[1], r4[2], r4[3]);
                        *reinterpret_cast<float4*>(gates + gs + base) = make_float4(z4[0], z4[1], z4[2], z4[3]);
                        *reinterpret_cast<float4*>(gates + 2 * gs + base) = make_float4(n4[0], n4[1], n4[2], n4[3]);
                        *reinterpret_cast<float4*>(gates + 3 * gs + base) = make_float4(hn4[0], hn4[1], hn4[2], hn4[3]);
                    }
                }
            }
        }
        __syncthreads();
        {
            const int rl = tid >> 2, part = tid & 3;
            float hacc[1 + LPG_Y];
#pragma unroll
            for (int c = 0; c < 1 + LPG_Y; ++c) hacc[c] = 0.0f;
            for (int k = part * 64; k < part * 64 + 64; ++k) {
                const float yv = fmax_nan(hB[rl * GF_HS + k], 0.0f);
                hacc[0] = fmaf(yv, swp[k], hacc[0]);
#pragma unroll
                for (int c = 0; c < LPG_Y; ++c) hacc[1 + c] = fmaf(yv, sWy[k * LPG_Y + c], hacc[1 + c]);
            }
#pragma unroll
            for (int c = 0; c < 1 + LPG_Y; ++c) {
                hacc[c] += __shfl_xor_sync(0xffffffffu, hacc[c], 1);
                hacc[c] += __shfl_xor_sync(0xffffffffu, hacc[c], 2);
            }
            if (part == 0 && rl < nrows) {
                const size_t tok = (size_t)t * R + row0 + rl;
                pi_hat[tok] = hacc[0] + b_pi;
                float zl[LPG_Y], pr[LPG_Y];
#pragma unroll
                for (int c = 0; c < LPG_Y; ++c) zl[c] = hacc[1 + c] + b_y[c];
                softmax_c<LPG_Y>(zl, pr);
                float4* yo = reinterpret_cast<float4*>(y_hat + tok * LPG_Y);
                yo[0] = make_float4(pr[0], pr[1], pr[2], pr[3]);
                yo[1] = make_float4(pr[4], pr[5], pr[6], pr[7]);
            }
        }
    }
}

static size_t gru_fwd_smem(int X) {
    return sizeof(float) * (2 * GF_TM * GF_HS + 2 * GF_KC * 192 + X * LPG_G + LPG_G + 2 * LPG_H +
                            LPG_H * LPG_Y + GF_TM * LPG_XP);
}

extern "C" int toued_gru_forward(const float* x, const uint8_t* done, const float* lpg_params, float* h_out,
                                 float* gates, float* pi_hat, float* y_hat, int n_agents, int n_workers,
                                 int rollout_len, int lifetime_conditioning, int lpg_stride, void* stream) {
    const int R = n_agents * n_workers;
    TOUED_CHECK(R > 0 && rollout_len > 0, "toued_gru_forward: empty problem");
    TOUED_CHECK(lpg_stride == 0 || n_workers % 64 == 0, "toued_gru_forward: per-agent parameters need n_workers %% 64 == 0");
    const int blocks = (R + GF_TM - 1) / GF_TM;
    cudaStream_t st = (cudaStream_t)stream;
    if (lifetime_conditioning) {
        const size_t smem = gru_fwd_smem(7);
        TOUED_CUDA(cudaFuncSetAttribute(gru_forward_kernel<7>, cudaFuncAttributeMaxDynamicSharedMemorySize, (int)smem));
        gru_forward_kernel<7><<<blocks, 256, smem, st>>>(x, done, lpg_params, h_out, gates, pi_hat, y_hat, R, rollout_len, n_workers, lpg_stride);
    } else {
        const size_t smem = gru_fwd_smem(5);
        TOUED_CUDA(cudaFuncSetAttribute(gru_forward_kernel<5>, cudaFuncAttributeMaxDynamicSharedMemorySize, (int)smem));
        gru_forward_kernel<5><<<blocks, 256, smem, st>>>(x, done, lpg_params, h_out, gates, pi_hat, y_hat, R, rollout_len, n_workers, lpg_stride);
    }
    TOUED_LAUNCH_CHECK();
    return 0;
}
```

to_ued_b200/meta/train.py:

```python
from __future__ import annotations

from typing import Any, Optional

import numpy as np
import torch

from .. import _lib
from ..util import prng
from ..util.data import AgentState, LpgHyperparams
from ..agents.lpg_agent import Tape, train_lpg_agent, train_lpg_agent_steps
from ..agents.agents import eval_agent
from ..environments.gridworld.gridworld import EnvState


class LPGTrainState:

    def __init__(self, model, params, tx, opt_state=None, step=0):
        self.model, self.params, self.tx = model, params, tx
        self.opt_state = tx.init(params) if opt_state is None else opt_state
        self.step = step

    def replace(self, **kw):
        d = dict(model=self.model, params=self.params, tx=self.tx, opt_state=self.opt_state, step=self.step)
        d.update(kw)
        return LPGTrainState(**d)


class MetaGradWorkspace:

    def __init__(self, n_agents, n_workers, rollout_len, obs_dim, num_updates, n_params, device):
        N, W, L, K = n_agents, n_workers, rollout_len, num_updates
        R = N * W
        f32 = torch.float32
        self.tape = Tape(N, W, L, obs_dim, K, device, keep_gates=True)
        self.d_pi_hat2 = [torch.empty((L, R), dtype=f32, device=device) for _ in range(2)]
        self.d_y_hat2 = [torch.empty((L, R, 8), dtype=f32, device=device) for _ in range(2)]
        self.dx2 = [torch.empty((L, R, 2), dtype=f32, device=device) for _ in range(2)]
        self.d_pi_hat, self.d_y_hat, self.dx = self.d_pi_hat2[0], self.d_y_hat2[0], self.dx2[0]
        self.dl2 = [torch.empty((L, R, 8), dtype=f32, device=device) for _ in range(2)]
        self.dl = self.dl2[0]
        self.lam = torch.empty((N, obs_dim, 8), dtype=f32, device=device)
        self.mu = torch.empty((N, obs_dim, 8), dtype=f32, device=device)
        self.whT = torch.empty((768, 256), dtype=f32, device=device)
        self.partials = torch.empty(_lib.lib().toued_lpg_wgrad_workspace_floats(), dtype=f32, device=device)
        self.loss_scal = torch.empty((N, 2), dtype=f32, device=device)
        self.ab_scratch = torch.empty(_lib.lib().toued_agent_scratch_floats(N, W, L, obs_dim), dtype=f32, device=device)
        if self.tape.precision == "tc":
            Rp = (R + 63) // 64 * 64
            self.whb_img = torch.empty(256 * 768, dtype=torch.float16, device=device)
            self.cotmax = torch.zeros((K, 2), dtype=torch.int32, device=device)
            self.dgimg2 = [torch.zeros(L * Rp * 1024 * 2, dtype=torch.uint8, device=device) for _ in range(2)]
            self.dgimg = self.dgimg2[0]
        self.off_small = _lib.lib().toued_lpg_wgrad_workspace_offset(1)
        self.key = (N, W, L, obs_dim, K, n_params, str(device))


_WS_CACHE = {}
_STREAMS = {}


def _workspace(n, w, L, D, K, P, device, slot=0) -> MetaGradWorkspace:
    import to_ued_b200
    key = (n, w, L, D, K, P, str(device), to_ued_b200.GRU_PRECISION)
    if _WS_CACHE and next(iter(_WS_CACHE))[:-1] != key:
        _WS_CACHE.clear()
    ws = _WS_CACHE.get(key + (slot,))
    if ws is None:
        ws = _WS_CACHE[key + (slot,)] = MetaGradWorkspace(n, w, L, D, K, P, device)
    return ws


def reverse_status(reset=False):
    st = torch.zeros((), dtype=torch.int32, device="cuda")
    for ws in _WS_CACHE.values():
        if getattr(ws, "cotmax", None) is not None:
            for w in ws.cotmax[:, 1]:
                st = st | w
            if reset:
                ws.cotmax[:, 1].zero_()
    return st


def _eval_stream(device):
    key = ("eval", str(device))
    if key not in _STREAMS:
        _STREAMS[key] = [torch.cuda.Stream(device=device)]
    return _STREAMS[key][0]


def _side_streams(device, n):
    key = str(device)
    lst = _STREAMS.setdefault(key, [])
    while len(lst) < n:
        lst.append(torch.cuda.Stream(device=device))
    return lst[:n]


def _world():
    import torch.distributed as dist
    if dist.is_available() and dist.is_initialized():
        return dist.get_world_size(), dist
    return 1, None


def lpg_meta_grad_train_step(rng, lpg_train_state: LPGTrainState, agent_states: AgentState, value_critic_states,
                             rollout_manager, num_mini_batches: int, gamma: float, gae_lambda: float,
                             lpg_hypers: LpgHyperparams, *, outer_product_quirk: bool = True,
                             global_agent_offset: int = 0, global_num_agents: Optional[int] = None,
                             eval_workers: int = 4, return_grad: bool = False, num_streams: Optional[int] = None,
                             _static: Optional[dict] = None):
    env = rollout_manager.env
    actor, critic = agent_states.actor_state, agent_states.critic_state
    N, W = agent_states.env_state.packed.shape
    L, K, D = rollout_manager.train_rollout_len, lpg_hypers.num_agent_updates, env.obs_dim
    dev = actor.params.device
    world, dist = _world()
    n_global = global_num_agents if global_num_agents is not None else N * world
    if dist is not None and global_num_agents is None:
        global_agent_offset = dist.get_rank() * N
    model = lpg_train_state.model
    cond = int(model.lifetime_conditioning)
    lpg = lpg_train_state.params
    P = lpg.numel()
    p, s = _lib.ptr, _lib.stream_ptr()

    rngs = prng.split_device(prng.to_device(rng, dev), n_global, global_agent_offset, N)[0]
    r_train, r_eval, r_evalagent = prng.chain_device(rngs, 3)

    if N % num_mini_batches != 0:
        raise ValueError(f"local agents ({N}) must be divisible by num_mini_batches ({num_mini_batches})")
    nb = N // num_mini_batches
    import to_ued_b200
    if num_streams is None:
        num_streams = to_ued_b200.NUM_STREAMS
    S = max(1, min(int(num_streams), num_mini_batches))
    wss = [_workspace(nb, W, L, D, K, P, dev, slot=i) for i in range(S)]
    main = torch.cuda.current_stream()
    streams = [main] if S == 1 else _side_streams(dev, S)
    tc = wss[0].tape.precision == "tc"
    gscale = 1.0 / n_global
    bK = [c / K for c in (lpg_hypers.policy_entropy_coeff, lpg_hypers.target_entropy_coeff,
                          lpg_hypers.policy_l2_coeff, lpg_hypers.target_l2_coeff)]
    if _static is not None:
        new_actor, new_critic, new_step, new_state, new_obs = _static["out"]
    else:
        new_actor = torch.empty_like(actor.params)
        new_critic = torch.empty_like(critic.params)
        new_step = torch.empty_like(actor.step)
        new_state = torch.empty_like(agent_states.env_state.packed)
        new_obs = torch.empty_like(agent_states.env_obs)
    msums = [torch.zeros(8, dtype=torch.float32, device=dev) for _ in range(S)]
    returns = torch.empty(N, dtype=torch.float32, device=dev)
    ready = torch.cuda.Event()
    ready.record(main)

    def _phase(label, chunk, stream):
        if to_ued_b200.PHASE_EVENTS is not None:
            e = torch.cuda.Event(enable_timing=True)
            e.record(stream)
            to_ued_b200.PHASE_EVENTS.append((label, chunk, e))
    _phase("start", -1, main)
    eval_done = [None] * S
    eval_stream = _side_streams(dev, S + 1)[S] if S > 1 else _eval_stream(dev)
    pool = _side_streams(dev, 5 * S + 1)
    ab_streams, em_streams = pool[S + 1:2 * S + 1], pool[2 * S + 1:3 * S + 1]
    ev_streams = [eval_stream] + pool[3 * S + 1:4 * S]
    wg_streams = pool[4 * S + 1:5 * S + 1]
    if not to_ued_b200.SIDE_STREAMS:
        ab_streams = em_streams = ev_streams = wg_streams = list(streams)
    evs = {}

    ctx, gens = {}, {}

    def forward_begin(mb):
        slot = mb % S
        ws, tape = wss[slot], wss[slot].tape
        with torch.cuda.stream(streams[slot]):
            if S > 1 and mb < S:
                streams[slot].wait_event(ready)
            if eval_done[slot] is not None:
                streams[slot].wait_event(eval_done[slot])
            sl = slice(mb * nb, (mb + 1) * nb)
            sub = AgentState(actor.replace(params=actor.params[sl], step=actor.step[sl]),
                             critic.replace(params=critic.params[sl], step=critic.step[sl]),
                             _sub_level(agent_states.level, sl), agent_states.env_obs[sl],
                             EnvState(agent_states.env_state.packed[sl], env.max_n_objs))
            levels = sub.level.packed
            gens[mb] = (train_lpg_agent_steps(r_train[sl], lpg_train_state, sub, rollout_manager, K,
                                              lpg_hypers.agent_target_coeff, tape=tape), sl, levels)
            next(gens[mb][0])

    def forward_step(mb):
        with torch.cuda.stream(streams[mb % S]):
            try:
                next(gens[mb][0])
            except StopIteration as fin:
                gens[mb] = (fin.value,) + gens[mb][1:]
            _phase("update", mb, streams[mb % S])

    def forward_end(mb):
        slot = mb % S
        ws, tape = wss[slot], wss[slot].tape
        res, sl, levels = gens.pop(mb)
        with torch.cuda.stream(streams[slot]):
            s = _lib.stream_ptr()
            if not isinstance(res, tuple):
                try:
                    while True:
                        next(res)
                except StopIteration as fin:
                    res = fin.value
            sub2, _, am = res
            state = sub2.env_state.packed
            _lib.call("toued_rollout", p(levels), p(r_eval[sl]), p(tape.actor[K]), None, p(state), p(tape.obs[K]),
                      p(tape.action[K]), p(tape.reward[K]), p(tape.done[K]), None, nb, W, L, D,
                      env.max_grid_size, env.max_n_objs, 0, s)
            _lib.call("toued_sort_tokens", p(tape.obs[K]), p(tape.sorted_tok[K]), nb, W, L, s)
            fwd_done = torch.cuda.Event()
            fwd_done.record(streams[slot])
            _phase("forward", mb, streams[slot])
            with torch.cuda.stream(ev_streams[slot]):
                ev_streams[slot].wait_event(fwd_done)
                returns[sl] = eval_agent(r_evalagent[sl], rollout_manager, levels, tape.actor[K], eval_workers)
                eval_done[slot] = torch.cuda.Event()
                eval_done[slot].record(ev_streams[slot])
            ctx[mb] = (sl, sub2, state, am, levels)

    def backward_begin(mb):
        slot = mb % S
        ws, tape = wss[slot], wss[slot].tape
        sl = ctx[mb][0]
        with torch.cuda.stream(streams[slot]):
            s = _lib.stream_ptr()
            if mb < S:
                if tc:
                    _lib.call("toued_pack_wh_backward", p(lpg), p(ws.whb_img), s)
                else:
                    _lib.call("toued_transpose_wh", p(lpg), p(ws.whT), s)
            vparams = value_critic_states.params[sl]
            _lib.call("toued_meta_loss", p(tape.obs[K]), p(tape.action[K]), p(tape.reward[K]), p(tape.done[K]),
                      p(tape.sorted_tok[K]), p(vparams), p(tape.actor[K]), p(ws.lam), p(ws.mu), p(ws.loss_scal),
                      nb, W, L, D, vparams.shape[-1], float(gamma), float(gae_lambda), float(gscale),
                      int(outer_product_quirk), s)
            evs[mb] = {"ml": torch.cuda.Event(), "ab": {}, "bwd": {}, "wg": {}, "em": {}}
            evs[mb]["ml"].record(streams[slot])

    def _agent_backward(ws, tape, k, buf, s):
        _lib.call("toued_agent_backward", p(tape.obs[k]), p(tape.action[k]), p(tape.sorted_tok[k]),
                  p(tape.pi_hat[k]), p(tape.y_hat[k]), p(tape.actor[k]), p(tape.critic[k]),
                  p(tape.actor[k + 1]), p(tape.critic[k + 1]), p(tape.scalars[k]), p(ws.lam), p(ws.mu),
                  p(ws.d_pi_hat2[buf]), p(ws.d_y_hat2[buf]), nb, W, L, D, float(actor.learning_rate),
                  float(critic.learning_rate), float(actor.max_grad_norm),
                  float(lpg_hypers.agent_target_coeff), *[float(b) for b in bK], float(gscale), p(ws.ab_scratch), s)

    def backward_step(mb, k):
        slot = mb % S
        ws, tape = wss[slot], wss[slot].tape
        first = (mb < S and k == K - 1)
        if not tc:
            with torch.cuda.stream(streams[slot]):
                s = _lib.stream_ptr()
                _agent_backward(ws, tape, k, 0, s)
                _lib.call("toued_gru_backward", p(tape.done[k]), p(lpg), p(ws.whT), p(tape.h[k]), p(tape.gates[k]),
                          p(tape.y_hat[k]), p(ws.d_pi_hat), p(ws.d_y_hat), p(ws.dl), p(ws.dx), nb, W, L, cond, s)
                _lib.call("toued_lpg_wgrad", p(tape.obs[k]), p(tape.done[k]), p(tape.critic[k]), p(lpg), p(tape.x[k]),
                          p(tape.h[k]), p(tape.gates[k]), p(ws.d_pi_hat), p(ws.dl), p(ws.dx), p(ws.partials),
                          nb, W, L, D, cond, 0 if first else 1, s)
            return
        ev, buf = evs[mb], k & 1
        for d in ("ab", "bwd", "wg", "em"):
            ev[d][k] = torch.cuda.Event()
        with torch.cuda.stream(ab_streams[slot]):
            st = ab_streams[slot]
            if k == K - 1:
                st.wait_event(ev["ml"])
            if k + 2 <= K - 1:
                st.wait_event(ev["wg"][k + 2])
            _agent_backward(ws, tape, k, buf, _lib.stream_ptr())
            _lib.call("toued_cotangent_max", p(ws.d_pi_hat2[buf]), p(ws.d_y_hat2[buf]), nb, W, L, p(ws.cotmax[k]),
                      _lib.stream_ptr())
            ev["ab"][k].record(st)
        with torch.cuda.stream(streams[slot]):
            st = streams[slot]
            s = _lib.stream_ptr()
            st.wait_event(ev["ab"][k])
            if k + 2 <= K - 1:
                st.wait_event(ev["em"][k + 2])
                st.wait_event(ev["wg"][k + 2])
            _lib.call("toued_gru_backward_tc", p(tape.done[k]), p(lpg), p(ws.whb_img), p(tape.h16[k]),
                      p(tape.fac[k]), p(tape.y_hat[k]), p(ws.d_pi_hat2[buf]), p(ws.d_y_hat2[buf]), p(ws.dgimg2[buf]), p(ws.dl2[buf]),
                      p(ws.dx2[buf]), p(ws.cotmax[k]), nb, W, L, cond, s)
            ev["bwd"][k].record(st)
            _phase(f"bwd{k}", mb, st)
        with torch.cuda.stream(wg_streams[slot]):
            st = wg_streams[slot]
            st.wait_event(ev["bwd"][k])
            _lib.call("toued_lpg_wgrad_tc", p(tape.hpimg[k]), p(ws.dgimg2[buf]), p(tape.ximg[k]), p(tape.h16[k]),
                      p(ws.d_pi_hat2[buf]), p(ws.dl2[buf]), p(ws.partials), p(ws.partials[ws.off_small:]),
                      p(ws.cotmax[k]), nb, W, L, 0 if first else 1, _lib.stream_ptr())
            ev["wg"][k].record(st)
            _phase(f"wgrad{k}", mb, st)
        with torch.cuda.stream(em_streams[slot]):
            st = em_streams[slot]
            st.wait_event(ev["bwd"][k])
            _lib.call("toued_lpg_wgrad_embed", p(tape.obs[k]), p(tape.done[k]), p(tape.critic[k]), p(lpg),
                      p(ws.dx2[buf]), p(ws.partials), p(ws.cotmax[k]), nb, W, L, D, cond, 0 if first else 1,
                      _lib.stream_ptr())
            ev["em"][k].record(st)

    def backward_end(mb):
        slot = mb % S
        ws, tape, msum = wss[slot], wss[slot].tape, msums[slot]
        sl, sub2, state, am, levels = ctx.pop(mb)
        with torch.cuda.stream(streams[slot]):
            ev = evs.pop(mb)
            if ev["em"]:
                streams[slot].wait_event(ev["em"][0])
                streams[slot].wait_event(ev["wg"][0])
            lpg_loss, value_loss = ws.loss_scal[:, 0], ws.loss_scal[:, 1]
            reg = (lpg_loss - lpg_hypers.policy_entropy_coeff * am.policy_entropy + lpg_hypers.policy_l2_coeff * am.policy_l2
                   - lpg_hypers.target_entropy_coeff * am.critic_entropy + lpg_hypers.target_l2_coeff * am.critic_l2)
            msum[:7] += torch.stack([lpg_loss.sum(), reg.sum(), value_loss.sum(), am.policy_l2.sum(),
                                     am.policy_entropy.sum(), am.critic_loss.sum(), am.critic_l2.sum()])
            msum[7] += am.critic_entropy.sum()
            new_actor[sl] = sub2.actor_state.params
            new_critic[sl] = sub2.critic_state.params
            new_step[sl] = sub2.actor_state.step
            new_state[sl] = state
            new_obs[sl] = tape.obs[K][:, -1]
            _phase("reverse_end", mb, streams[slot])

    for g0 in range(0, num_mini_batches, S):
        group = range(g0, min(num_mini_batches, g0 + S))
        for mb in group:
            forward_begin(mb)
            forward_step(mb)
        for k in range(1, K):
            for mb in group:
                forward_step(mb)
        for mb in group:
            forward_end(mb)
        for mb in group:
            backward_begin(mb)
        for k in reversed(range(K)):
            for mb in group:
                backward_step(mb, k)
        for mb in group:
            backward_end(mb)
    for st in ([] if S == 1 else list(streams)) + ev_streams:
        ev = torch.cuda.Event()
        ev.record(st)
        main.wait_event(ev)
    s = _lib.stream_ptr()
    msum = msums[0] if S == 1 else torch.stack(msums).sum(0)

    grad = torch.empty(P, dtype=torch.float32, device=dev)
    L_ = _lib.lib()
    n_wh, n_sm = (L_.toued_wgrad_tc_splits(), L_.toued_wgrad_tc_small_splits()) if tc else \
        (L_.toued_lpg_wgrad_splits(0), L_.toued_lpg_wgrad_splits(1))
    _lib.call("toued_reduce_partials", p(wss[0].partials), p(grad), cond, n_wh, n_sm, s)
    for ws in wss[1:min(S, num_mini_batches)]:
        g2 = torch.empty_like(grad)
        _lib.call("toued_reduce_partials", p(ws.partials), p(g2), cond, n_wh, n_sm, s)
        grad += g2
    red = torch.cat([grad, msum, returns.sum().view(1)])
    if dist is not None:
        dist.all_reduce(red)
    grad, mvec = red[:P], red[P:] / n_global
    if _static is not None:
        ost = lpg_train_state.opt_state
        lpg_train_state.tx.update_dev_(lpg, grad, ost["mu"], ost["nu"], _static["count_dev"])
        new_lpg = lpg_train_state
    else:
        new_params = lpg.clone()
        opt_state = lpg_train_state.tx.update_(new_params, grad, {**lpg_train_state.opt_state,
                                                                  "mu": lpg_train_state.opt_state["mu"].clone(),
                                                                  "nu": lpg_train_state.opt_state["nu"].clone()})
        new_lpg = lpg_train_state.replace(params=new_params, opt_state=opt_state, step=lpg_train_state.step + 1)
    agent_out = agent_states.replace(
        actor_state=actor.replace(params=new_actor, step=new_step),
        critic_state=critic.replace(params=new_critic, step=new_step if _static is not None else new_step.clone()),
        env_obs=new_obs, env_state=EnvState(new_state, env.max_n_objs),
        host_step=_advance_host_step(agent_states.host_step, agent_states.level.lifetime, K))
    if _static is not None:
        value_critic_states.step.add_(K + 1)
        value_out = value_critic_states
    else:
        value_out = value_critic_states.replace(step=value_critic_states.step + (K + 1))
    metrics = {
        "lpg_loss": mvec[0], "reg_lpg_loss": mvec[1], "value_loss": mvec[2],
        "lpg_agent": {"policy_l2": mvec[3], "policy_entropy": mvec[4], "critic_loss": mvec[5],
                      "critic_l2": mvec[6], "critic_entropy": mvec[7]},
        "lpg_agent_return": mvec[8],
    }
    if return_grad:
        metrics["_grad"] = grad
    if _static is not None:
        metrics["_mvec"] = mvec
    _phase("end", -1, main)
    return new_lpg, agent_out, value_out, metrics


def _advance_host_step(step, lifetime, k):
    if step is None:
        return None
    return np.minimum(step + k, np.maximum(step, lifetime)).astype(np.int32)


def _sub_level(level, sl):
    from ..util.data import Level
    return Level(level.env_params, level.lifetime[sl], level.buffer_id[sl], level.packed[sl])
```

Measured before the change: 469.0 million.

## Record tabular softmax outputs in forward and reuse them in update and backward

lpg_prepare and agent_update now write per-token unnormalized softmax numerators plus inverse sums for the actor and critic tables into a 15-plane record. agent_update and agent_backward read these records instead of recomputing the table logits and softmax from the gathered table rows. This trades gather-plus-exp arithmetic for extra global memory writes and reads of 15 floats per token, and adds tape memory. A build variant keeps the recompute path available.

```diff
diff --git a/__graft_entry__.py b/__graft_entry__.py
--- a/__graft_entry__.py
+++ b/__graft_entry__.py
@@ -10,6 +10,7 @@
     from to_ued_b200.csrc.build import build as _build
     path = _build(verbose=False)
     _build(verbose=False, variant="fuzz")
+    _build(verbose=False, variant="tabrecompute")
     import to_ued_b200
     from to_ued_b200 import _lib
     assert os.path.exists(path) and _lib.lib().toued_version() >= 1
diff --git a/include/toued.h b/include/toued.h
--- a/include/toued.h
+++ b/include/toued.h
@@ -31,6 +31,11 @@
                       const float* lpg_params, const int32_t* step, const void* levels, float* x,
                       void* ximg, int n_agents, int n_workers, int rollout_len, int obs_dim,
                       int lifetime_conditioning, int lpg_stride, void* stream);
+int toued_lpg_prepare_rec(const int32_t* obs, const uint8_t* action, const float* reward,
+                          const uint8_t* done, const float* actor, const float* critic,
+                          const float* lpg_params, const int32_t* step, const void* levels, float* x,
+                          void* ximg, float* tab_rec, int n_agents, int n_workers, int rollout_len, int obs_dim,
+                          int lifetime_conditioning, int lpg_stride, void* stream);
 
 int toued_gru_forward(const float* x, const uint8_t* done, const float* lpg_params, float* h_out,
                       float* gates, float* pi_hat, float* y_hat, int n_agents, int n_workers,
@@ -38,8 +43,8 @@
 
 int toued_agent_scratch_floats(int n_agents, int n_workers, int rollout_len, int obs_dim);
 int toued_agent_update(const int32_t* obs, const uint8_t* action, const uint16_t* sorted_tok,
-                       const float* pi_hat, const float* y_hat, const float* actor_in,
-                       const float* critic_in, float* actor_out, float* critic_out,
+                       const float* pi_hat, const float* y_hat, const float* tab_rec_k, float* tab_rec_k1,
+                       const float* actor_in, const float* critic_in, float* actor_out, float* critic_out,
                        const void* levels, int32_t* step, float* scalars, int n_agents,
                        int n_workers, int rollout_len, int obs_dim, float lr_actor, float lr_critic,
                        float max_grad_norm, float agent_target_coeff, int tables_precopied, float* run_scratch,
@@ -53,7 +58,8 @@
                     float gae_lambda, float grad_scale, int outer_product_quirk, void* stream);
 
 int toued_agent_backward(const int32_t* obs, const uint8_t* action, const uint16_t* sorted_tok,
-                         const float* pi_hat, const float* y_hat, const float* actor_k,
+                         const float* pi_hat, const float* y_hat, const float* tab_rec_k,
+                         const float* tab_rec_k1, const float* actor_k,
                          const float* critic_k, const float* actor_k1, const float* critic_k1,
                          const float* update_scalars, float* lam, float* mu, float* d_pi_hat,
                          float* d_y_hat, int n_agents, int n_workers, int rollout_len, int obs_dim,
diff --git a/to_ued_b200/_lib.py b/to_ued_b200/_lib.py
--- a/to_ued_b200/_lib.py
+++ b/to_ued_b200/_lib.py
@@ -34,11 +34,12 @@
     "toued_env_reset": [_P] * 3 + [_I] * 3 + [_P],
     "toued_sort_tokens": [_P] * 2 + [_I] * 3 + [_P],
     "toued_lpg_prepare": [_P] * 11 + [_I] * 6 + [_P],
+    "toued_lpg_prepare_rec": [_P] * 12 + [_I] * 6 + [_P],
     "toued_gru_forward": [_P] * 7 + [_I] * 5 + [_P],
-    "toued_agent_update": [_P] * 12 + [_I] * 4 + [_F] * 4 + [_I, _P, _P],
+    "toued_agent_update": [_P] * 14 + [_I] * 4 + [_F] * 4 + [_I, _P, _P],
     "toued_agent_scratch_floats": [_I] * 4,
     "toued_meta_loss": [_P] * 10 + [_I] * 5 + [_F] * 3 + [_I, _P],
-    "toued_agent_backward": [_P] * 14 + [_I] * 4 + [_F] * 9 + [_P, _P],
+    "toued_agent_backward": [_P] * 16 + [_I] * 4 + [_F] * 9 + [_P, _P],
     "toued_transpose_wh": [_P] * 3,
     "toued_gru_backward": [_P] * 10 + [_I] * 4 + [_P],
     "toued_lpg_wgrad_workspace_floats": [],
diff --git a/to_ued_b200/agents/lpg_agent.py b/to_ued_b200/agents/lpg_agent.py
--- a/to_ued_b200/agents/lpg_agent.py
+++ b/to_ued_b200/agents/lpg_agent.py
@@ -64,6 +64,8 @@
             self.gates = torch.empty((ka, 4, L, R, 256), dtype=f32, device=dev) if self.record else None
         self.pi_hat = torch.empty((ka, L, R), dtype=f32, device=dev)
         self.y_hat = torch.empty((ka, L, R, 8), dtype=f32, device=dev)
+        self.tab_rec = torch.empty((ka, 15, L, R), dtype=f32, device=dev)
+        self.tab_rec1 = torch.empty((ka, 15, L, R), dtype=f32, device=dev) if self.record else None
         self.scalars = torch.empty((ka, N, 8), dtype=f32, device=dev)
         self.scal_sum = torch.zeros((N, 8), dtype=f32, device=dev)
         self.step_in = torch.empty((ka, N), dtype=i32, device=dev)
@@ -124,9 +126,9 @@
         ev_sort.record(side)
     _mark("rollout")
     tape.step_in[a].copy_(step)
-    _lib.call("toued_lpg_prepare", p(tape.obs[r]), p(tape.action[r]), p(tape.reward[r]), p(tape.done[r]),
+    _lib.call("toued_lpg_prepare_rec", p(tape.obs[r]), p(tape.action[r]), p(tape.reward[r]), p(tape.done[r]),
               p(tape.actor[t0]), p(tape.critic[t0]), p(lpg_params), p(step), p(levels), p(tape.x[a]),
-              p(tape.ximg[a]) if tape.ximg is not None else None,
+              p(tape.ximg[a]) if tape.ximg is not None else None, p(tape.tab_rec[a]),
               N, W, L, D, int(lifetime_conditioning), int(lpg_stride), s)
     if lpg_stride and tape.precision == "tc":
         _lib.call("toued_gru_forward_tc_multi", p(tape.x[a]), p(tape.done[r]), p(lpg_params), p(tape.wh_img),
@@ -144,7 +146,7 @@
     cur.wait_event(ev_sort)
     _mark("sort_wait")
     _lib.call("toued_agent_update", p(tape.obs[r]), p(tape.action[r]), p(tape.sorted_tok[r]), p(tape.pi_hat[a]),
-              p(tape.y_hat[a]), p(tape.actor[t0]), p(tape.critic[t0]), p(tape.actor[t1]), p(tape.critic[t1]),
+              p(tape.y_hat[a]), p(tape.tab_rec[a]), p(tape.tab_rec1[a]) if tape.record else None, p(tape.actor[t0]), p(tape.critic[t0]), p(tape.actor[t1]), p(tape.critic[t1]),
               p(levels), p(step), p(tape.scalars[a]), N, W, L, D, float(lr_actor), float(lr_critic),
               float(max_grad_norm), float(agent_target_coeff), int(precopied), p(tape.agent_scratch), s)
     tape.scal_sum += tape.scalars[a]
diff --git a/to_ued_b200/csrc/agent_backward.cu b/to_ued_b200/csrc/agent_backward.cu
--- a/to_ued_b200/csrc/agent_backward.cu
+++ b/to_ued_b200/csrc/agent_backward.cu
@@ -134,13 +134,12 @@
 
 struct TokFwd { float p[5], y[8], pa, q, tf; int a; };
 
-__device__ __forceinline__ TokFwd tok_forward(const float* at, const float* ct, int D, int32_t o, int a) {
+template <bool REC>
+__device__ __forceinline__ TokFwd tok_forward(const float* rec, size_t plane, size_t li, const float* at,
+                                              const float* ct, int D, int32_t o, int a) {
     TokFwd f;
-    float z[5], zy[8];
-    tab_logits8<5>(at, D, o, z);
-    softmax_c<5>(z, f.p);
-    tab_logits8<8>(ct, D, o, zy);
-    softmax_c<8>(zy, f.y);
+    if (REC) tab_rec_read(rec, plane, li, at, ct, D, o, f.p, f.y);
+    else tab_eval(at, ct, D, o, f.p, f.y);
     f.a = a;
     f.pa = f.p[0];
 #pragma unroll
@@ -173,7 +172,8 @@
 __global__ void __launch_bounds__(256, 2)
 agent_backward_kernel(const int32_t* __restrict__ obs, const uint8_t* __restrict__ action,
                       const uint16_t* __restrict__ sorted_tok, const float* __restrict__ pi_hat,
-                      const float* __restrict__ y_hat, const float* __restrict__ actor_k,
+                      const float* __restrict__ y_hat, const float* __restrict__ rec_k,
+                      const float* __restrict__ rec_k1, const float* __restrict__ actor_k,
                       const float* __restrict__ critic_k, const float* __restrict__ actor_k1,
                       const float* __restrict__ critic_k1, const float* __restrict__ upd_scal,
                       float* lam, float* mu, float* __restrict__ d_pi_hat, float* __restrict__ d_y_hat,
@@ -195,6 +195,7 @@
     float* lm = lam + (size_t)n * D * 8;
     float* mm = mu + (size_t)n * D * 8;
     const float invT = 1.0f / (float)T;
+    const size_t plane = (size_t)L * R;
     const float gna = upd_scal[n * 8 + 0], gnc = upd_scal[n * 8 + 1];
     const bool keep = upd_scal[n * 8 + 2] != 0.0f;
     float* runv = run_scratch + (size_t)n * min(T, D) * 13;
@@ -205,7 +206,9 @@
 #pragma unroll
     for (int j = 0; j < 13; ++j) last[j] = 0.f;
     for (int tok = tid; tok < T; tok += 256) {
-        const TokFwd f = tok_forward(a1, c1, D, ob[tok], act[tok]);
+        const int t = tok / W, w = tok - t * W;
+        const size_t li = (size_t)t * R + (size_t)n * W + w;
+        const TokFwd f = tok_forward<true>(rec_k1, plane, li, a1, c1, D, ob[tok], act[tok]);
         float* r = rec + tok * 13;
         {
             float dh[5], s = 0.f;
@@ -266,7 +269,7 @@
     for (int tok = tid; tok < T; tok += 256) {
         const int t = tok / W, w = tok - t * W;
         const size_t li = (size_t)t * R + (size_t)n * W + w;
-        const TokFwd f = tok_forward(a0, c0, D, ob[tok], act[tok]);
+        const TokFwd f = tok_forward<true>(rec_k, plane, li, a0, c0, D, ob[tok], act[tok]);
         float yh[8]; load8(y_hat + li * 8, yh);
         float* r = rec + tok * 13;
         tok_grad(f, pi_hat[li], yh, invT, alpha, r);
@@ -327,7 +330,7 @@
         const int tok = si.tok[pos];
         const int t = tok / W, w = tok - t * W;
         const size_t li = (size_t)t * R + (size_t)n * W + w;
-        const TokFwd f = tok_forward(a0, c0, D, ob[tok], act[tok]);
+        const TokFwd f = tok_forward<false>(rec_k, plane, li, a0, c0, D, ob[tok], act[tok]);
         const float ph = pi_hat[li];
         float yh[8]; load8(y_hat + li * 8, yh);
         float* r = rec + tok * 13;
@@ -395,7 +398,8 @@
 }
 
 extern "C" int toued_agent_backward(const int32_t* obs, const uint8_t* action, const uint16_t* sorted_tok,
-                                    const float* pi_hat, const float* y_hat, const float* actor_k,
+                                    const float* pi_hat, const float* y_hat, const float* tab_rec_k,
+                                    const float* tab_rec_k1, const float* actor_k,
                                     const float* critic_k, const float* actor_k1, const float* critic_k1,
                                     const float* update_scalars, float* lam, float* mu, float* d_pi_hat,
                                     float* d_y_hat, int n_agents, int n_workers, int rollout_len, int obs_dim,
@@ -406,13 +410,14 @@
     const int T = n_workers * rollout_len;
     TOUED_CHECK(n_agents > 0 && T > 0, "toued_agent_backward: empty problem");
     TOUED_CHECK(run_scratch != nullptr, "toued_agent_backward: run_scratch (toued_agent_scratch_floats) is required");
+    TOUED_CHECK(tab_rec_k != nullptr && tab_rec_k1 != nullptr, "toued_agent_backward: the tabular forward records are required");
     const size_t smem = sizeof(float) * ((size_t)T * 13 + 2 * 256 * 13) + seg_index_bytes(T);
     TOUED_CHECK(smem <= 200 * 1024, "toued_agent_backward: W*L=%d too large for shared memory", T);
     TOUED_CUDA(cudaFuncSetAttribute(agent_backward_kernel, cudaFuncAttributeMaxDynamicSharedMemorySize, (int)smem));
     TOUED_CUDA(cudaFuncSetAttribute(agent_backward_kernel, cudaFuncAttributePreferredSharedMemoryCarveout, 100));
     cudaStream_t st = (cudaStream_t)stream;
     agent_backward_kernel<<<n_agents, 256, smem, st>>>(
-        obs, action, sorted_tok, pi_hat, y_hat, actor_k, critic_k, actor_k1, critic_k1, update_scalars, lam, mu,
+        obs, action, sorted_tok, pi_hat, y_hat, tab_rec_k, tab_rec_k1, actor_k, critic_k, actor_k1, critic_k1, update_scalars, lam, mu,
         d_pi_hat, d_y_hat, run_scratch, n_agents, n_workers, rollout_len, obs_dim, lr_actor, lr_critic, max_grad_norm,
         agent_target_coeff, policy_entropy_coeff, target_entropy_coeff, policy_l2_coeff, target_l2_coeff, grad_scale);
     TOUED_LAUNCH_CHECK();
diff --git a/to_ued_b200/csrc/agent_update.cu b/to_ued_b200/csrc/agent_update.cu
--- a/to_ued_b200/csrc/agent_update.cu
+++ b/to_ued_b200/csrc/agent_update.cu
@@ -7,7 +7,8 @@
 __global__ void __launch_bounds__(256, 2)
 agent_update_kernel(const int32_t* __restrict__ obs, const uint8_t* __restrict__ action,
                     const uint16_t* __restrict__ sorted_tok, const float* __restrict__ pi_hat,
-                    const float* __restrict__ y_hat, const float* __restrict__ actor_in,
+                    const float* __restrict__ y_hat, const float* __restrict__ rec_k, float* __restrict__ rec_k1,
+                    const float* __restrict__ actor_in,
                     const float* __restrict__ critic_in, float* actor_out, float* critic_out,
                     const LevelRec* __restrict__ levels, int32_t* __restrict__ step,
                     float* __restrict__ scal, float* run_scratch, int n_agents, int W, int L, int D,
@@ -27,6 +28,7 @@
     float* a_out = actor_out + (size_t)n * D * 8;
     float* c_out = critic_out + (size_t)n * D * 8;
     const float invT = 1.0f / (float)T;
+    const size_t plane = (size_t)L * R;
     const SegIndex si = seg_index_build(idxmem, iscan, sorted_tok + (size_t)n * T, ob, T);
 
     if (!tables_precopied)
@@ -43,11 +45,8 @@
         const int t = tok / W, w = tok - t * W;
         const size_t li = (size_t)t * R + (size_t)n * W + w;
         const int32_t o = ob[tok];
-        float z[5], p[5], zy[8], y[8];
-        tab_logits8<5>(a_in, D, o, z);
-        softmax_c<5>(z, p);
-        tab_logits8<8>(c_in, D, o, zy);
-        softmax_c<8>(zy, y);
+        float p[5], y[8];
+        tab_rec_read(rec_k, plane, li, a_in, c_in, D, o, p, y);
         const int a = act[tok];
         float pa = p[0];
 #pragma unroll
@@ -122,12 +121,19 @@
 
     float ea = 0.f, ec = 0.f;
     for (int tok = tid; tok < T; tok += 256) {
+        const int t = tok / W, w = tok - t * W;
         const int32_t o = ob[tok];
-        float z[5], p[5], zy[8], y[8];
+        float z[5], p[5], zy[8], y[8], ia, iy;
         tab_logits8<5>(a_out, D, o, z);
-        softmax_c<5>(z, p);
+        softmax_num<5>(z, p, ia);
         tab_logits8<8>(c_out, D, o, zy);
-        softmax_c<8>(zy, y);
+        softmax_num<8>(zy, y, iy);
+        if (rec_k1)
+            tab_rec_store(rec_k1, plane, (size_t)t * R + (size_t)n * W + w, p, ia, y, iy);
+#pragma unroll
+        for (int j = 0; j < 5; ++j) p[j] *= ia;
+#pragma unroll
+        for (int j = 0; j < 8; ++j) y[j] *= iy;
 #pragma unroll
         for (int j = 0; j < 5; ++j) { const float q = p[j] + 1e-8f; ea -= q * logf(q); }
 #pragma unroll
@@ -150,7 +156,8 @@
 }
 
 extern "C" int toued_agent_update(const int32_t* obs, const uint8_t* action, const uint16_t* sorted_tok,
-                                  const float* pi_hat, const float* y_hat, const float* actor_in,
+                                  const float* pi_hat, const float* y_hat, const float* tab_rec_k, float* tab_rec_k1,
+                                  const float* actor_in,
                                   const float* critic_in, float* actor_out, float* critic_out,
                                   const void* levels, int32_t* step, float* scalars, int n_agents,
                                   int n_workers, int rollout_len, int obs_dim, float lr_actor,
@@ -164,9 +171,10 @@
     TOUED_CUDA(cudaFuncSetAttribute(agent_update_kernel, cudaFuncAttributeMaxDynamicSharedMemorySize, (int)smem));
     TOUED_CUDA(cudaFuncSetAttribute(agent_update_kernel, cudaFuncAttributePreferredSharedMemoryCarveout, 100));
     TOUED_CHECK(run_scratch != nullptr, "toued_agent_update: run_scratch (toued_agent_scratch_floats) is required");
+    TOUED_CHECK(tab_rec_k != nullptr, "toued_agent_update: tab_rec_k (written by toued_lpg_prepare_rec) is required");
     cudaStream_t st = (cudaStream_t)stream;
     agent_update_kernel<<<n_agents, 256, smem, st>>>(
-        obs, action, sorted_tok, pi_hat, y_hat, actor_in, critic_in, actor_out, critic_out,
+        obs, action, sorted_tok, pi_hat, y_hat, tab_rec_k, tab_rec_k1, actor_in, critic_in, actor_out, critic_out,
         (const LevelRec*)levels, step, scalars, run_scratch, n_agents, n_workers, rollout_len, obs_dim,
         lr_actor, lr_critic, max_grad_norm, agent_target_coeff, tables_precopied);
     TOUED_LAUNCH_CHECK();
diff --git a/to_ued_b200/csrc/build.py b/to_ued_b200/csrc/build.py
--- a/to_ued_b200/csrc/build.py
+++ b/to_ued_b200/csrc/build.py
@@ -26,6 +26,7 @@
     "fwd1": ["-DFT_HEADS_WARP=0"],
     "pf2": ["-DBT_PF_DEPTH=2"],
     "pf": ["-DBT_L2_PREFETCH=1"],
+    "tabrecompute": ["-DTOUED_TAB_RECOMPUTE=1"],
     "old": ["-DTOUED_XTILE_OLD=1"],
     "probe_old": ["-DTOUED_RACE_PROBE=1", "-DTOUED_XTILE_OLD=1"],
 }
diff --git a/to_ued_b200/csrc/lpg_common.cuh b/to_ued_b200/csrc/lpg_common.cuh
--- a/to_ued_b200/csrc/lpg_common.cuh
+++ b/to_ued_b200/csrc/lpg_common.cuh
@@ -48,14 +48,20 @@
 }
 
 template <int C>
-__device__ __forceinline__ void softmax_c(const float (&z)[C], float (&p)[C]) {
+__device__ __forceinline__ void softmax_num(const float (&z)[C], float (&e)[C], float& inv) {
     float m = z[0];
 #pragma unroll
     for (int j = 1; j < C; ++j) m = fmaxf(m, z[j]);
     float s = 0.0f;
 #pragma unroll
-    for (int j = 0; j < C; ++j) { p[j] = __expf(z[j] - m); s += p[j]; }
-    const float inv = 1.0f / s;
+    for (int j = 0; j < C; ++j) { e[j] = __expf(z[j] - m); s += e[j]; }
+    inv = 1.0f / s;
+}
+
+template <int C>
+__device__ __forceinline__ void softmax_c(const float (&z)[C], float (&p)[C]) {
+    float inv;
+    softmax_num<C>(z, p, inv);
 #pragma unroll
     for (int j = 0; j < C; ++j) p[j] *= inv;
 }
@@ -73,6 +79,44 @@
     for (int j = 0; j < C; ++j) z[j] = r[j] + tf * l[j];
 }
 
+constexpr int TAB_REC = 15;
+
+__device__ __forceinline__ void tab_rec_store(float* __restrict__ rec, size_t plane, size_t li, const float (&ea)[5],
+                                              float ia, const float (&ey)[8], float iy) {
+#pragma unroll
+    for (int j = 0; j < 5; ++j) rec[j * plane + li] = ea[j];
+    rec[5 * plane + li] = ia;
+#pragma unroll
+    for (int j = 0; j < 8; ++j) rec[(6 + j) * plane + li] = ey[j];
+    rec[14 * plane + li] = iy;
+}
+
+__device__ __forceinline__ void tab_eval(const float* at, const float* ct, int D, int32_t o, float (&p)[5], float (&y)[8]) {
+    float z[5], zy[8];
+    tab_logits8<5>(at, D, o, z);
+    softmax_c<5>(z, p);
+    tab_logits8<8>(ct, D, o, zy);
+    softmax_c<8>(zy, y);
+}
+
+__device__ __forceinline__ void tab_rec_read(const float* __restrict__ rec, size_t plane, size_t li, const float* at,
+                                             const float* ct, int D, int32_t o, float (&p)[5], float (&y)[8]) {
+#if TOUED_TAB_RECOMPUTE
+    tab_eval(at, ct, D, o, p, y);
+#else
+#pragma unroll
+    for (int j = 0; j < 5; ++j) p[j] = __ldg(rec + j * plane + li);
+    const float ia = __ldg(rec + 5 * plane + li);
+#pragma unroll
+    for (int j = 0; j < 8; ++j) y[j] = __ldg(rec + (6 + j) * plane + li);
+    const float iy = __ldg(rec + 14 * plane + li);
+#pragma unroll
+    for (int j = 0; j < 5; ++j) p[j] *= ia;
+#pragma unroll
+    for (int j = 0; j < 8; ++j) y[j] *= iy;
+#endif
+}
+
 __device__ __forceinline__ float block_sum(float v, float* red) {
 #pragma unroll
     for (int o = 16; o > 0; o >>= 1) v += __shfl_xor_sync(0xffffffffu, v, o);
diff --git a/to_ued_b200/csrc/lpg_forward.cu b/to_ued_b200/csrc/lpg_forward.cu
--- a/to_ued_b200/csrc/lpg_forward.cu
+++ b/to_ued_b200/csrc/lpg_forward.cu
@@ -130,7 +130,7 @@
                    const float* __restrict__ actor, const float* __restrict__ critic,
                    const float* __restrict__ lpg, const int32_t* __restrict__ step,
                    const LevelRec* __restrict__ levels, float* __restrict__ x, unsigned char* __restrict__ ximg,
-                   int n_agents, int W, int L, int D, int cond, int emb_off, int lpg_stride) {
+                   float* __restrict__ tabrec, int n_agents, int W, int L, int D, int cond, int emb_off, int lpg_stride) {
     __shared__ float sp_s[LPG_Y * LPG_E + LPG_E + LPG_E + 1];
     if (lpg_stride == 0) {
         for (int i = threadIdx.x; i < LPG_Y * LPG_E + 2 * LPG_E + 1; i += blockDim.x) sp_s[i] = lpg[emb_off + i];
@@ -147,23 +147,29 @@
     const int32_t ob1 = obs[((size_t)n * (L + 1) + t + 1) * W + w];
     const float* at = actor + (size_t)n * D * 8;
     const float* ct = critic + (size_t)n * D * 8;
-    float z[TOUED_NUM_ACTIONS], p[TOUED_NUM_ACTIONS];
+    const size_t row = (size_t)n * W + w;
+    float z[TOUED_NUM_ACTIONS], p[TOUED_NUM_ACTIONS], ia;
     tab_logits8<TOUED_NUM_ACTIONS>(at, D, ob, z);
-    softmax_c<TOUED_NUM_ACTIONS>(z, p);
+    softmax_num<TOUED_NUM_ACTIONS>(z, p, ia);
+    float zy[LPG_Y], y0[LPG_Y], y1[LPG_Y], iy;
+    tab_logits8<LPG_Y>(ct, D, ob, zy);
+    softmax_num<LPG_Y>(zy, y0, iy);
+    if (tabrec)
+        tab_rec_store(tabrec, (size_t)L * n_agents * W, (size_t)t * n_agents * W + row, p, ia, y0, iy);
+#pragma unroll
+    for (int j = 0; j < TOUED_NUM_ACTIONS; ++j) p[j] *= ia;
+#pragma unroll
+    for (int j = 0; j < LPG_Y; ++j) y0[j] *= iy;
     const int a = action[g];
     float pa = p[0];
 #pragma unroll
     for (int j = 1; j < TOUED_NUM_ACTIONS; ++j) pa = (a == j) ? p[j] : pa;
-    float zy[LPG_Y], y0[LPG_Y], y1[LPG_Y];
-    tab_logits8<LPG_Y>(ct, D, ob, zy);
-    softmax_c<LPG_Y>(zy, y0);
     tab_logits8<LPG_Y>(ct, D, ob1, zy);
     softmax_c<LPG_Y>(zy, y1);
     const float d = done[g] ? 1.0f : 0.0f;
     float pyt, pyt1;
     embed_mlp2(y0, y1, sp, pyt, pyt1);
     pyt1 *= (1.0f - d);
-    const size_t row = (size_t)n * W + w;
     float4* xo = reinterpret_cast<float4*>(x + ((size_t)t * n_agents * W + row) * LPG_XP);
     xo[0] = make_float4(reward[g], d, pa + 1e-8f, pyt);
     const float4 v1 = make_float4(pyt1, cond ? (float)step[n] : 0.0f, cond ? (float)levels[n].lifetime : 0.0f, 1.0f);
@@ -179,19 +185,28 @@
     }
 }
 
+extern "C" int toued_lpg_prepare_rec(const int32_t* obs, const uint8_t* action, const float* reward,
+                                     const uint8_t* done, const float* actor, const float* critic,
+                                     const float* lpg_params, const int32_t* step, const void* levels,
+                                     float* x, void* ximg, float* tab_rec, int n_agents, int n_workers, int rollout_len,
+                                     int obs_dim, int lifetime_conditioning, int lpg_stride, void* stream) {
+    const size_t total = (size_t)n_agents * rollout_len * n_workers;
+    TOUED_CHECK(total > 0, "toued_lpg_prepare: empty problem");
+    lpg_prepare_kernel<<<(unsigned)((total + 255) / 256), 256, 0, (cudaStream_t)stream>>>(
+        obs, action, reward, done, actor, critic, lpg_params, step, (const LevelRec*)levels, x, (unsigned char*)ximg,
+        (float*)tab_rec, n_agents, n_workers, rollout_len, obs_dim, lifetime_conditioning,
+        lpg_offsets(lifetime_conditioning ? 7 : 5).e_w0, lpg_stride);
+    TOUED_LAUNCH_CHECK();
+    return 0;
+}
+
 extern "C" int toued_lpg_prepare(const int32_t* obs, const uint8_t* action, const float* reward,
                                  const uint8_t* done, const float* actor, const float* critic,
                                  const float* lpg_params, const int32_t* step, const void* levels,
                                  float* x, void* ximg, int n_agents, int n_workers, int rollout_len, int obs_dim,
                                  int lifetime_conditioning, int lpg_stride, void* stream) {
-    const size_t total = (size_t)n_agents * rollout_len * n_workers;
-    TOUED_CHECK(total > 0, "toued_lpg_prepare: empty problem");
-    lpg_prepare_kernel<<<(unsigned)((total + 255) / 256), 256, 0, (cudaStream_t)stream>>>(
-        obs, action, reward, done, actor, critic, lpg_params, step, (const LevelRec*)levels, x, (unsigned char*)ximg,
-        n_agents, n_workers, rollout_len, obs_dim, lifetime_conditioning,
-        lpg_offsets(lifetime_conditioning ? 7 : 5).e_w0, lpg_stride);
-    TOUED_LAUNCH_CHECK();
-    return 0;
+    return toued_lpg_prepare_rec(obs, action, reward, done, actor, critic, lpg_params, step, levels, x, ximg, nullptr,
+                                 n_agents, n_workers, rollout_len, obs_dim, lifetime_conditioning, lpg_stride, stream);
 }
 
 constexpr int GF_TM = 64;
diff --git a/to_ued_b200/meta/train.py b/to_ued_b200/meta/train.py
--- a/to_ued_b200/meta/train.py
+++ b/to_ued_b200/meta/train.py
@@ -247,7 +247,7 @@
 
     def _agent_backward(ws, tape, k, buf, s):
         _lib.call("toued_agent_backward", p(tape.obs[k]), p(tape.action[k]), p(tape.sorted_tok[k]),
-                  p(tape.pi_hat[k]), p(tape.y_hat[k]), p(tape.actor[k]), p(tape.critic[k]),
+                  p(tape.pi_hat[k]), p(tape.y_hat[k]), p(tape.tab_rec[k]), p(tape.tab_rec1[k]), p(tape.actor[k]), p(tape.critic[k]),
                   p(tape.actor[k + 1]), p(tape.critic[k + 1]), p(tape.scalars[k]), p(ws.lam), p(ws.mu),
                   p(ws.d_pi_hat2[buf]), p(ws.d_y_hat2[buf]), nb, W, L, D, float(actor.learning_rate),
                   float(critic.learning_rate), float(actor.max_grad_norm),
```

Result: no change. 469.2 million, median of 6 (+0.0%).
